# fbcotter/pytorch_wavelets

Hardware: AMD Instinct MI355X
Metric: Mpixels/s fwd+inv DWT J=3 db4, Nx3x512x512 fp32; % HBM roofline (higher is better)
Workload: dtype f32; 1 GPU; DWTForward+DWTInverse J=3 db4 symmetric, 128x3x512x512 fp32 per GPU (BASELINE configs[1]); global_batch=128, parallelism=batch-sharded x1, no data-path collective, step=forward + inverse

## Files before the change

include/wavelets_hip.h:

```cpp
#ifndef WAVELETS_HIP_H
#define WAVELETS_HIP_H
#include <stdint.h>

#ifdef __cplusplus
extern "C" {
#endif

#define WL_F32 0
#define WL_F16 1
#define WL_F64 2
#define WL_BF16 3

#define WL_ERR_MODE (-1)
#define WL_ERR_SHAPE (-2)
#define WL_ERR_UNSUPPORTED (-3)
#define WL_ERR_DTYPE (-4)
#define WL_ERR_TAPS (-5)
#define WL_MAX_TAPS 128

int wl_version(void);
const char* wl_backend(void);

int wl_set_option(const char* name, int value);
int wl_get_option(const char* name);
const char* wl_last_kernel(void);
long long wl_launch_count(void);
long long wl_last_grid(void);
const char* wl_kernel_history(int back);

int wl_dwt_coeff_len(int n, int L, int mode);

int wl_dwt2d_analysis(const void* x, void* ll, void* highs, int dtype, int64_t planes, int H, int W,
                      const void* h_w_lo, const void* h_w_hi, int Lw,
                      const void* h_h_lo, const void* h_h_hi, int Lh, int mode, void* stream);

int wl_dwt2d_analysis_strided(const void* x, int64_t x_plane_stride, int x_row_stride, void* ll,
                              int64_t ll_plane_stride, int ll_row_stride, void* highs, int dtype, int64_t planes,
                              int H, int W, const void* h_w_lo, const void* h_w_hi, int Lw, const void* h_h_lo,
                              const void* h_h_hi, int Lh, int mode, void* stream);

int wl_dwt2d_synthesis(const void* ll, int64_t ll_plane_stride, int ll_row_stride, const void* highs,
                       void* y, int dtype, int64_t planes, int Kh, int Kw, int OH, int OW,
                       const void* g_w_lo, const void* g_w_hi, int Lw,
                       const void* g_h_lo, const void* g_h_hi, int Lh, int mode, void* stream);

int wl_dwt2d_analysis_fused(const void* x, void* yl, void* const* yh, int dtype, int64_t planes, int H,
                            int W, int nlev, const void* h_w_lo, const void* h_w_hi, const void* h_h_lo,
                            const void* h_h_hi, int L, int mode, int strips, void* stream);
int wl_dwt2d_analysis_fused_ex(const void* x, int64_t x_plane_stride, int x_row_stride, void* yl, void* const* yh,
                               int dtype, int64_t planes, int H, int W, int nlev, const void* h_w_lo,
                               const void* h_w_hi, const void* h_h_lo, const void* h_h_hi, int L, int mode,
                               int strips, void* tap_scratch, int* tap_state, void* stream);

int wl_dwt2d_synthesis_fused(const void* yl, int64_t yl_plane_stride, int yl_row_stride, int yl_h, int yl_w,
                             const void* const* yh, const int* Kh, const int* Kw, void* y, int dtype,
                             int64_t planes, int nlev, const void* g_w_lo, const void* g_w_hi,
                             const void* g_h_lo, const void* g_h_hi, int L, int mode, int strips, void* stream);
int wl_dwt2d_synthesis_fused_ex(const void* yl, int64_t yl_plane_stride, int yl_row_stride, int yl_h, int yl_w,
                                const void* const* yh, const int* Kh, const int* Kw, void* y, int dtype,
                                int64_t planes, int nlev, const void* g_w_lo, const void* g_w_hi,
                                const void* g_h_lo, const void* g_h_hi, int L, int mode, int strips, void* tap_scratch,
                                int* tap_state, void* stream);

int wl_dwt2d_analysis_nonsep(const void* x, void* y, int dtype, int64_t planes, int H, int W, const void* f,
                             int Ly, int Lx, int mode, void* stream);
int wl_dwt2d_synthesis_nonsep(const void* coeffs, void* y, int dtype, int64_t planes, int Kh, int Kw, int OH,
                              int OW, const void* g, int Ly, int Lx, int mode, void* stream);


int wl_dtcwt_fwd_level1(const void* x, void* ll, void* highs, int dtype, int64_t planes, int H, int W,
                        const void* h0, int L0, const void* h1, int L1, int mode, void* stream);

int wl_dtcwt_fwd_level2(const void* x, void* ll, void* highs, int dtype, int64_t planes, int H, int W,
                        const void* h0a, const void* h0b, const void* h1a, const void* h1b, int L, void* stream);

int wl_dtcwt_fwd_level12(const void* x, void* highs1, void* ll2, void* highs2, int dtype, int64_t planes, int H, int W,
                         const void* h0o, int L0, const void* h1o, int L1, const void* h0a, const void* h0b,
                         const void* h1a, const void* h1b, int LQ, int mode, int policy, void* stream);

int wl_dtcwt_inv_level21(const void* ll2, int64_t ll2_plane_stride, int ll2_row_stride, const void* highs2,
                         const void* highs1, void* y, int dtype, int64_t planes, int H, int W, const void* g0o, int L0,
                         const void* g1o, int L1, const void* g0a, const void* g0b, const void* g1a, const void* g1b, int LQ,
                         int mode, int policy, void* stream);

int wl_dtcwt_inv_level1(const void* ll, int64_t ll_plane_stride, int ll_row_stride, const void* highs, void* y,
                        int dtype, int64_t planes, int H, int W, const void* g0, int L0, const void* g1, int L1,
                        int mode, void* stream);

int wl_dtcwt_inv_level2(const void* ll, int64_t ll_plane_stride, int ll_row_stride, const void* highs, void* y,
                        int dtype, int64_t planes, int h, int w, const void* g0a, const void* g0b, const void* g1a,
                        const void* g1b, int L, void* stream);

int wl_scat_fwd_level1(const void* x, void* z, void* drdx, void* drdy, void* ll, int dtype, int64_t N, int C, int H,
                       int W, const void* h0, int L0, const void* h1, int L1, int mode, double magbias,
                       int combine_colour, void* stream);

int wl_scat_fwd_level1_into(const void* x, void* z, int64_t z_batch_stride, int64_t z_ll_offset, int64_t z_mag_offset,
                            void* ll, int dtype, int64_t N, int C, int H, int W, const void* h0, int L0, const void* h1,
                            int L1, int mode, double magbias, void* stream);
int wl_scat_fwd_level2_into(const void* x, void* z, int64_t z_batch_stride, int64_t z_ll_offset, int64_t z_mag_offset,
                            int dtype, int64_t N, int C, int H, int W, const void* h0a, const void* h0b, const void* h1a,
                            const void* h1b, int L, double magbias, void* stream);

int wl_scat_bwd_level1(const void* dz, const void* drdx, const void* drdy, void* dx, int dtype, int64_t N, int C,
                       int H, int W, const void* h0, int L0, const void* h1, int L1, int mode, int combine_colour,
                       void* stream);

#define WL_TAP_SCRATCH_BYTES 64
int wl_dwt2d_analysis_stream(const void* x, int64_t x_plane_stride, int x_row_stride, void* ll, int64_t ll_plane_stride,
                             int ll_row_stride, void* highs, int dtype, int64_t planes, int H, int W, const void* h_w_lo,
                             const void* h_w_hi, const void* h_h_lo, const void* h_h_hi, int L, int mode, int policy,
                             void* stream);
int wl_dwt2d_analysis_stream_ex(const void* x, int64_t x_plane_stride, int x_row_stride, void* ll, int64_t ll_plane_stride,
                                int ll_row_stride, void* highs, int dtype, int64_t planes, int H, int W, const void* h_w_lo,
                                const void* h_w_hi, const void* h_h_lo, const void* h_h_hi, int L, int mode, int policy,
                                void* tap_scratch, int* tap_state, void* stream);

int wl_dwt2d_synthesis_stream(const void* ll, int64_t ll_plane_stride, int ll_row_stride, const void* highs, void* y,
                              int dtype, int64_t planes, int Kh, int Kw, int OH, int OW, const void* g_w_lo,
                              const void* g_w_hi, const void* g_h_lo, const void* g_h_hi, int L, int mode, int policy,
                              void* stream);
int wl_dwt2d_synthesis_stream_ex(const void* ll, int64_t ll_plane_stride, int ll_row_stride, const void* highs, void* y,
                                 int dtype, int64_t planes, int Kh, int Kw, int OH, int OW, const void* g_w_lo,
                                 const void* g_w_hi, const void* g_h_lo, const void* g_h_hi, int L, int mode, int policy,
                                 void* tap_scratch, int* tap_state, void* stream);

int wl_dwt2d_analysis_nonsep_bwd(const void* dy, void* dx, int dtype, int64_t planes, int H, int W, const void* f,
                                 int Ly, int Lx, int mode, void* stream);
int wl_dwt2d_synthesis_nonsep_bwd(const void* dy, void* dc, int dtype, int64_t planes, int Kh, int Kw, const void* g,
                                  int Ly, int Lx, int mode, void* stream);

int wl_dwt1d_analysis_fused(const void* x, void* lo, void* const* highs, int dtype, int64_t rows, int N, int J,
                            const void* h0, const void* h1, int L, int mode, void* stream);

int wl_dwt1d_synthesis_fused(const void* lo, int n_lo, const void* const* highs, const int* n_hi, void* y, int out_len, int dtype,
                             int64_t rows, int J, const void* g0, const void* g1, int L, int mode, void* stream);

int wl_corr1d(const void* x, void* y0, void* y1, int dtype, int64_t outer, int n, int64_t inner, int64_t y_outer_stride,
              int K, const void* h0, const void* h1, int tap_offset, int tap_stride, int ntaps, int start, int step,
              int tap_step, int ext, int out_offset, int out_stride, void* stream);

int wl_dwt2d_analysis_small(const void* x, void* yl, void* const* yh, int dtype, int64_t planes, int H, int W, int nlev,
                            const void* h_w_lo, const void* h_w_hi, const void* h_h_lo, const void* h_h_hi, int L, int mode,
                            void* stream);

int wl_dwt2d_synthesis_small(const void* yl, int yl_h, int yl_w, const void* const* yh, const int* Kh, const int* Kw, void* y,
                             int dtype, int64_t planes, int nlev, const void* g_w_lo, const void* g_w_hi, const void* g_h_lo,
                             const void* g_h_hi, int L, int mode, void* stream);

int wl_dtcwt_fwd_level1_rot(const void* x, void* ll, void* re, void* im, int dtype, int64_t N, int C, int H, int W,
                            const void* h0, int L0, const void* h1, int L1, const void* h2, int L2, int mode,
                            int scat, double magbias, void* stream);

int wl_swt2d_level(const void* x, int64_t x_ps, void* y, int dtype, int64_t planes, int H, int W,
                   const void* h_w_lo, const void* h_w_hi, const void* h_h_lo, const void* h_h_hi, int Lw, int Lh,
                   int dilation, int ext, void* stream);

int wl_iswt2d_level(const void* y, int64_t y_ps, const void* ll, int64_t ll_ps, int ll_mode, void* x, int dtype, int64_t planes,
                    int H, int W, const void* h_w_lo, const void* h_w_hi, const void* h_h_lo, const void* h_h_hi, int Lw, int Lh,
                    int dilation, int ext, double scale, void* stream);

int wl_corr1d_adj(const void* y0, int64_t y0_outer_stride, const void* y1, int64_t y1_outer_stride, void* dx, int dtype,
                  int64_t outer, int n, int64_t inner, int K, const void* h0, const void* h1, int ntaps, int start, int tap_step,
                  int ext, double scale, void* stream);

int wl_synth1d(const void* lo, const void* hi, void* y, int dtype, int64_t outer, int K, int64_t inner, int ny,
               const void* g0, const void* g1, int L, int mode, void* stream);

#ifdef __cplusplus
}
#endif
#endif
```

pytorch_wavelets_amd/_capi.py:

```python
import ctypes as C

P = C.c_void_p
I = C.c_int
L = C.c_int64

PROTOTYPES = {
    'wl_version': (I, []),
    'wl_backend': (C.c_char_p, []),
    'wl_set_option': (I, [C.c_char_p, I]),
    'wl_get_option': (I, [C.c_char_p]),
    'wl_last_kernel': (C.c_char_p, []),
    'wl_launch_count': (C.c_longlong, []),
    'wl_last_grid': (C.c_longlong, []),
    'wl_kernel_history': (C.c_char_p, [I]),
    'wl_dwt_coeff_len': (I, [I, I, I]),
    'wl_dwt2d_analysis': (I, [P, P, P, I, L, I, I, P, P, I, P, P, I, I, P]),
    'wl_dwt2d_analysis_strided': (I, [P, L, I, P, L, I, P, I, L, I, I, P, P, I, P, P, I, I, P]),
    'wl_dwt2d_synthesis': (I, [P, L, I, P, P, I, L, I, I, I, I, P, P, I, P, P, I, I, P]),
    'wl_dwt2d_analysis_fused': (I, [P, P, C.POINTER(P), I, L, I, I, I, P, P, P, P, I, I, I, P]),
    'wl_dwt2d_analysis_fused_ex': (I, [P, L, I, P, C.POINTER(P), I, L, I, I, I, P, P, P, P, I, I, I, P, C.POINTER(I), P]),
    'wl_dwt2d_synthesis_fused': (I, [P, L, I, I, I, C.POINTER(P), C.POINTER(I), C.POINTER(I), P, I, L, I, P, P, P, P, I, I, I, P]),
    'wl_dwt2d_synthesis_fused_ex': (I, [P, L, I, I, I, C.POINTER(P), C.POINTER(I), C.POINTER(I), P, I, L, I, P, P, P, P, I, I, I, P, C.POINTER(I), P]),
    'wl_dwt2d_analysis_stream': (I, [P, L, I, P, L, I, P, I, L, I, I, P, P, P, P, I, I, I, P]),
    'wl_dwt2d_analysis_stream_ex': (I, [P, L, I, P, L, I, P, I, L, I, I, P, P, P, P, I, I, I, P, C.POINTER(I), P]),
    'wl_dwt2d_synthesis_stream': (I, [P, L, I, P, P, I, L, I, I, I, I, P, P, P, P, I, I, I, P]),
    'wl_dwt2d_synthesis_stream_ex': (I, [P, L, I, P, P, I, L, I, I, I, I, P, P, P, P, I, I, I, P, C.POINTER(I), P]),
    'wl_dwt2d_analysis_nonsep': (I, [P, P, I, L, I, I, P, I, I, I, P]),
    'wl_dwt2d_synthesis_nonsep': (I, [P, P, I, L, I, I, I, I, P, I, I, I, P]),
    'wl_dwt2d_analysis_nonsep_bwd': (I, [P, P, I, L, I, I, P, I, I, I, P]),
    'wl_dwt2d_synthesis_nonsep_bwd': (I, [P, P, I, L, I, I, P, I, I, I, P]),
    'wl_dtcwt_fwd_level1': (I, [P, P, P, I, L, I, I, P, I, P, I, I, P]),
    'wl_dtcwt_fwd_level2': (I, [P, P, P, I, L, I, I, P, P, P, P, I, P]),
    'wl_dtcwt_fwd_level12': (I, [P, P, P, P, I, L, I, I, P, I, P, I, P, P, P, P, I, I, I, P]),
    'wl_dtcwt_inv_level21': (I, [P, L, I, P, P, P, I, L, I, I, P, I, P, I, P, P, P, P, I, I, I, P]),
    'wl_dtcwt_inv_level1': (I, [P, L, I, P, P, I, L, I, I, P, I, P, I, I, P]),
    'wl_dtcwt_inv_level2': (I, [P, L, I, P, P, I, L, I, I, P, P, P, P, I, P]),
    'wl_scat_fwd_level1': (I, [P, P, P, P, P, I, L, I, I, I, P, I, P, I, I, C.c_double, I, P]),
    'wl_scat_fwd_level1_into': (I, [P, P, L, L, L, P, I, L, I, I, I, P, I, P, I, I, C.c_double, P]),
    'wl_scat_fwd_level2_into': (I, [P, P, L, L, L, I, L, I, I, I, P, P, P, P, I, C.c_double, P]),
    'wl_dwt1d_analysis_fused': (I, [P, P, C.POINTER(P), I, L, I, I, P, P, I, I, P]),
    'wl_dwt2d_analysis_small': (I, [P, P, C.POINTER(P), I, L, I, I, I, P, P, P, P, I, I, P]),
    'wl_dwt2d_synthesis_small': (I, [P, I, I, C.POINTER(P), C.POINTER(I), C.POINTER(I), P, I, L, I, P, P, P, P, I, I, P]),
    'wl_dtcwt_fwd_level1_rot': (I, [P, P, P, P, I, L, I, I, I, P, I, P, I, P, I, I, I, C.c_double, P]),
    'wl_swt2d_level': (I, [P, L, P, I, L, I, I, P, P, P, P, I, I, I, I, P]),
    'wl_iswt2d_level': (I, [P, L, P, L, I, P, I, L, I, I, P, P, P, P, I, I, I, I, C.c_double, P]),
    'wl_dwt1d_synthesis_fused': (I, [P, I, C.POINTER(P), C.POINTER(I), P, I, I, L, I, P, P, I, I, P]),
    'wl_corr1d': (I, [P, P, P, I, L, I, L, L, I, P, P, I, I, I, I, I, I, I, I, I, P]),
    'wl_corr1d_adj': (I, [P, L, P, L, P, I, L, I, L, I, P, P, I, I, I, I, C.c_double, P]),
    'wl_synth1d': (I, [P, P, P, I, L, I, L, I, P, P, I, I, P]),
    'wl_scat_bwd_level1': (I, [P, P, P, P, I, L, I, I, I, P, I, P, I, I, I, P]),
}


def bind(lib):
    for name, (res, args) in PROTOTYPES.items():
        fn = getattr(lib, name)
        fn.restype = res
        fn.argtypes = args
    return lib
```

pytorch_wavelets_amd/csrc/wl_api_common.h:

```cpp
#pragma once
#include <stdlib.h>
#include "../../include/wavelets_hip.h"
#include "wl_common.h"
#include "wl_lattice.h"

static int wl_mode_to_ext(int mode) {
    switch (mode) {
        case 0: return WL_EXT_ZERO;
        case 1: return WL_EXT_SYM;
        case 2: return WL_EXT_PER;
        case 4: return WL_EXT_REFL;
        case 6: return WL_EXT_PERIODIC;
        default: return -1;
    }
}

static inline int wl_coeff_len(int n, int L, int mode) { return mode == 2 ? (n + 1) / 2 : (n + L - 1) / 2; }

static int wl_afb_base(int n, int L, int mode) {
    if (mode == 2) return L / 2 - L + 1;
    const int K = (n + L - 1) / 2;
    const int p = 2 * (K - 1) - n + L;
    return -(p / 2);
}

struct WlBanks { const void* w_lo; const void* w_hi; const void* h_lo; const void* h_hi; };
struct WlAfbReq {
    const void* x; int64_t x_ps; int x_rs;
    void* ll; int64_t ll_ps; int ll_rs; void* highs;
    int64_t planes; int H, W;
    WlBanks taps; int Lw, Lh, mode;
    int policy; float* scratch; int* tstate; void* stream;
};
struct WlSfbReq {
    const void* ll; int64_t ll_ps; int ll_rs; const void* highs; void* y;
    int64_t planes; int Kh, Kw, OH, OW;
    WlBanks taps; int Lw, Lh, mode;
    int policy; float* scratch; int* tstate; void* stream;
};
struct WlAfbPyrReq {
    const void* x; int64_t x_ps; int x_rs;
    void* yl; void* const* yh;
    int64_t planes; int H, W, nlev;
    WlBanks taps; int L, mode;
    int strips, hints; float* scratch; int* tstate; void* stream;
};
struct WlSfbPyrReq {
    const void* yl; int64_t yl_ps; int yl_rs; int yl_h, yl_w;
    const void* const* yh; const int* Kh; const int* Kw; void* y;
    int64_t planes; int nlev;
    WlBanks taps; int L, mode;
    int strips, hints; float* scratch; int* tstate; void* stream;
};

#define WL_DISPATCH_DTYPE(dtype, ...)                      \
    switch (dtype) {                                       \
        case WL_F32: { typedef float T; __VA_ARGS__; } break;    \
        case WL_F16: { typedef wl_half T; __VA_ARGS__; } break;  \
        case WL_BF16: { typedef wl_bf16 T; __VA_ARGS__; } break; \
        case WL_F64: { typedef double T; __VA_ARGS__; } break;   \
        default: return WL_ERR_DTYPE;                      \
    }
#define WL_DISPATCH_FLOAT(dtype, ...)                                      \
    do {                                                                   \
        if ((dtype) == WL_F32) { typedef float T; __VA_ARGS__; }           \
        if ((dtype) == WL_F16) { typedef wl_half T; __VA_ARGS__; }         \
        if ((dtype) == WL_BF16) { typedef wl_bf16 T; __VA_ARGS__; }        \
        return (dtype) == WL_F64 ? WL_ERR_UNSUPPORTED : WL_ERR_DTYPE;      \
    } while (0)

#define WL_GUARDED_PAIR(HINT, PLAIN, ...)                         \
    do {                                                          \
        int rc_ = PLAIN(__VA_ARGS__, 2, 1);                       \
        if (rc_ != 0) return rc_;                                 \
        rc_ = HINT(__VA_ARGS__, 1, 0);                            \
        if (rc_ != 0) return rc_;                                 \
        return PLAIN(__VA_ARGS__, 2, 2);                          \
    } while (0)

template <int LT, typename Plain, typename Lattice>
static int wl_lattice_launch(Plain plain, Lattice lattice, const WlBanks& b, int syn, int same, size_t elem_size,
                             float* scratch, int* tstate, int bits, void* stream) {
    int rc = plain(2, 1);
    if (rc != 0) return rc;
    rc = lattice(1, 1);
    if (rc != 0) return rc;
    WlTapPrepArgs p;
    p.h_w_lo = (const float*)b.w_lo; p.h_w_hi = (const float*)b.w_hi; p.h_h_lo = (const float*)b.h_lo; p.h_h_hi = (const float*)b.h_hi;
    p.out = scratch; p.L = LT; p.syn = syn; p.same = same;
    p.tol = elem_size == 2 ? 0x1p-12f : 0x1p-22f;
    rc = wl_tap_examined(tstate, bits) ? 0 : wl_launch_aux<WlTapPrep<LT> >(p, 1, 0, stream);
    if (rc != 0) return rc;
    wl_tap_mark(tstate, bits);
    rc = lattice(1, 0);
    if (rc != 0) return rc;
    return plain(2, 2);
}
```

pytorch_wavelets_amd/csrc/wl_idwt_rows.h:

```cpp
#pragma once
#include "wl_common.h"
#include "wl_dwt_rows.h"
#include "wl_lattice.h"

#define WL_IROWS_MAXLEV 3
#define WL_IROWS_WAVES 14
#define WL_IROWS_MAXHB 640
#ifndef WL_IROWS_ABLATE
#define WL_IROWS_ABLATE 0
#endif
#if (WL_IROWS_ABLATE & 8) && defined(__HIPCC__)
#define WL_ITICK() __builtin_readcyclecounter()
#else
#define WL_ITICK() 0ull
#endif
#define WL_IROWS_CHUNK 1024

struct WlIRowsLevel {
    int Kh, Kw;
    int OH, OW;
    int src_off[4];
    int ll_rows;
    int ll_pitch;
    int rbytes;
    int dma_rows;
    int dma_shift;
    int cpr;
    int nwaves;
    int per_d0, head_off;
    int per_grp;
};

struct WlIRowsSeg {
    int nhb;
    int f0[WL_IROWS_MAXLEV], fend[WL_IROWS_MAXLEV];
    int rho[WL_IROWS_MAXLEV];
    int own_lo, own_hi;
    unsigned sched[WL_IROWS_MAXHB / 4];
};

template <typename T>
struct WlIRowsArgs {
    const T* yl;
    const T* yh[WL_IROWS_MAXLEV];
    T* y;
    const float* g_w_lo;
    const float* g_w_hi;
    const float* g_h_lo;
    const float* g_h_hi;
    int64_t NC, ll_ps;
    int nlev, nwhole, lds_bytes;
    signed char role_level[WL_IROWS_WAVES];
    short role_arg[WL_IROWS_WAVES];
    signed char role_sub[WL_IROWS_WAVES];
    int pp, lds_plane;
    WlIRowsLevel g[WL_IROWS_MAXLEV];
    WlIRowsSeg seg[3];
    int per;
    int guard;
    const float* lat;
};

struct WlIRowsSched {
    int fed[WL_IROWS_MAXLEV];
    WL_HD void init(const WlIRowsSeg& sg) { for (int j = 0; j < WL_IROWS_MAXLEV; ++j) fed[j] = sg.f0[j]; }
    WL_HD int made(const WlIRowsSeg& sg, int j, int LT) const {
        const int warm = (LT - 2) / 2;
        return fed[j] - sg.f0[j] > warm ? 2 * (fed[j] - warm) : 2 * sg.f0[j];
    }
    template <typename A> WL_HD int feeds_now(const A& a, const WlIRowsSeg& sg, int j, int LT) const {
        const int warm = (LT - 2) / 2;
        int n = 0;
        while (n < 2 && fed[j] + n < sg.fend[j]) {
            const int k = fed[j] + n;
            if (j + 1 < a.nlev && k >= made(sg, j + 1, LT) && !(a.per && k >= a.g[j].Kh)) break;
            if (j > 0 && k - sg.f0[j] >= warm && 2 * (k - warm) + 1 - a.g[j - 1].ll_rows >= fed[j - 1]) break;
            ++n;
        }
        return n;
    }
};

#ifndef WL_IROWS_LAT_MIN
#define WL_IROWS_LAT_MIN 8
#endif
template <typename T, int LT, int LAT = 0, int PER = 0>
struct WlSfbRows {
    typedef WlIRowsArgs<T> Args;
    static const int kThreads = 64 * WL_IROWS_WAVES;
    static const int kMinWaves = 7;
    static const int HL = LT / 2;
    static const int WARM = HL - 1;
    static const int SZ = (int)sizeof(T);

    static WL_DEV void loader(const Args& a, const WlIRowsSeg& sg, const WlCtx& ctx, int64_t plane, int lane, int j, int s0, int ns, int soff) {
        const WlIRowsLevel& g = a.g[j];
        const int rb = g.rbytes, R = g.dma_rows, cpr = g.cpr;
        const int plane_bytes = g.Kh * rb, ring_bytes = R * rb;
        const int f0 = sg.f0[j], fend = sg.fend[j];
        const int r0 = f0 >> g.dma_shift;
        const char* src[4];
        int dst[4];
#pragma unroll
        for (int i = 0; i < 4; ++i) {
            const int s = s0 + (i < ns ? i : 0);
            src[i] = s == 0 ? reinterpret_cast<const char*>(a.yl + (size_t)plane * a.ll_ps)
                            : reinterpret_cast<const char*>(a.yh[j] + ((size_t)plane * 3 + (s - 1)) * ((size_t)g.Kh * g.Kw));
            dst[i] = g.src_off[s] + soff;
        }
        auto need = [&](int k) { return ((k >> g.dma_shift) - r0) * cpr + (((k & (R - 1)) + 1) * rb - 1) / WL_IROWS_CHUNK + 1; };
        const int total = fend > f0 ? need(fend - 1) : 0;
        const int max_steps = WL_IROWS_MAX_VM / ns - 1;
        const int p16 = plane_bytes & ~15, ptail = (plane_bytes & 15) / 4;
        int issued = 0, landed = 0;
        int r = r0, c = 0;
        int rbyte = 0, pbyte = r0 * ring_bytes;
        int fed = f0;
        auto try_issue = [&]() {
            if (issued >= total || issued - landed >= max_steps) return false;
            const int cend = rbyte + WL_IROWS_CHUNK < ring_bytes ? rbyte + WL_IROWS_CHUNK : ring_bytes;
            if (r != r0 && cend > (fed - 2 - (r - 1) * R) * rb) return false;
            if (!(WL_IROWS_ABLATE & 2)) {
                const bool whole = pbyte + 16 <= plane_bytes;
                const bool on = rbyte + lane * 16 < ring_bytes && pbyte + lane * 16 + 16 <= plane_bytes;
                const bool tail = ptail && p16 >= pbyte && p16 < pbyte + (cend - rbyte);
#pragma unroll
                for (int i = 0; i < 4; ++i) {
                    if (i >= ns) break;
                    if (whole) wl_dma16_s(ctx, (unsigned)(dst[i] + rbyte), src[i], (unsigned)(pbyte + lane * 16), on);
                    if (tail) wl_dma4_s(ctx, (unsigned)(dst[i] + rbyte + (p16 - pbyte)), src[i], (unsigned)(p16 + lane * 4), lane < ptail);
                }
            }
            ++issued;
            rbyte += WL_IROWS_CHUNK; pbyte += WL_IROWS_CHUNK;
            if (++c == cpr) { c = 0; ++r; rbyte = 0; pbyte = r * ring_bytes; }
            return true;
        };
        while (try_issue()) {}
        unsigned long long tw = 0, tb = 0, ti = 0;
        unsigned word = sg.sched[0];
        for (int hb = 0; hb < sg.nhb; ++hb) {
            const unsigned long long c0 = WL_ITICK();
            const int n = (int)(word >> (8 * (hb & 3) + 2 * j)) & 3;
            if ((hb & 3) == 3) word = sg.sched[(hb >> 2) + 1 < WL_IROWS_MAXHB / 4 ? (hb >> 2) + 1 : 0];
            if (n) {
                const int nd = need(fed + n - 1);
                if (issued < nd) wl_fail();
                if (!(WL_IROWS_ABLATE & 2)) wl_wait_vm_dyn((issued - nd) * ns);
                landed = nd;
            }
            const unsigned long long c1 = WL_ITICK();
            if (!(WL_IROWS_ABLATE & 64) || !(hb & 1)) ctx.sync();
            const unsigned long long c2 = WL_ITICK();
            fed += n;
            while (try_issue()) {}
            tw += c1 - c0; tb += c2 - c1; ti += WL_ITICK() - c2;
        }
        wl_wait_vm<0>();
        if ((WL_IROWS_ABLATE & 8) && lane == 0) {
            T* o = a.y + (size_t)plane * a.g[0].OH * a.g[0].OW + 4 * (ctx.tid >> 6);
            o[0] = (T)(float)(tw >> 6); o[1] = (T)(float)(tb >> 6); o[2] = (T)(float)(ti >> 6);
        }
    }

    static WL_DEV void loader_per(const Args& a, const WlIRowsSeg& sg, const WlCtx& ctx, int64_t plane, int lane, int j, int s0, int ns, int soff) {
        const WlIRowsLevel& g = a.g[j];
        const int P = g.rbytes, R = g.dma_rows, Kh = g.Kh, rowb = g.Kw * SZ;
        const int rowb16 = rowb & ~15, tail = (rowb & 15) / 4;
        const int nseg = (rowb16 + WL_IROWS_CHUNK - 1) / WL_IROWS_CHUNK;
        const int per_row = ns * (nseg + (tail ? 1 : 0));
        const int f0 = sg.f0[j], fend = sg.fend[j], rho = sg.rho[j];
        const char* src[4];
        int dst[4];
#pragma unroll
        for (int i = 0; i < 4; ++i) {
            const int s = s0 + (i < ns ? i : 0);
            src[i] = s == 0 ? reinterpret_cast<const char*>(a.yl + (size_t)plane * a.ll_ps)
                            : reinterpret_cast<const char*>(a.yh[j] + ((size_t)plane * 3 + (s - 1)) * ((size_t)g.Kh * g.Kw));
            dst[i] = g.src_off[s] + soff;
        }
        const int G = g.per_grp;
        const int per_step = G > 1 ? ns : per_row;
        const int lrg = (16 * lane) / P, lo = 16 * lane - lrg * P - g.per_d0;
        const bool lon = lrg < G && lo >= 0 && lo + 16 <= rowb;
        const int fend_g = (fend + G - 1) & ~(G - 1);
        const int max_rows = (WL_IROWS_MAX_VM / per_step - 1) * G;
        int next = f0, landed = f0;
        int fed = f0;
        auto try_issue = [&]() {
            if (next >= fend_g || next - landed >= max_rows) return false;
            if (next + G - 1 - R >= fed - 2) return false;
            if (G > 1) {
                int sr = next + lrg - WARM + rho;
                sr = sr < 0 ? sr + Kh : sr;
                sr = sr >= Kh ? sr - Kh : sr;
                sr = sr >= Kh ? sr - Kh : sr;
                const unsigned gro = (unsigned)sr * (unsigned)rowb + (unsigned)lo;
                const unsigned slot = (unsigned)((next & (R - 1)) * P);
                if (!(WL_IROWS_ABLATE & 2)) {
#pragma unroll
                    for (int i = 0; i < 4; ++i) {
                        if (i >= ns) break;
                        wl_dma16_s(ctx, (unsigned)dst[i] + slot, src[i], gro, lon);
                    }
                }
                next += G;
                return true;
            }
            int sr = next - WARM + rho;
            sr = sr < 0 ? sr + Kh : sr;
            sr = sr >= Kh ? sr - Kh : sr;
            const unsigned gro = (unsigned)sr * (unsigned)rowb;
            const unsigned slot = (unsigned)((next & (R - 1)) * P + g.per_d0);
            if (!(WL_IROWS_ABLATE & 2)) {
#pragma unroll
                for (int i = 0; i < 4; ++i) {
                    if (i >= ns) break;
                    for (int q = 0; q < nseg; ++q) {
                        const int byte = (q * 64 + lane) * 16;
                        wl_dma16_s(ctx, (unsigned)dst[i] + slot + (unsigned)(q * WL_IROWS_CHUNK), src[i], gro + (unsigned)byte, byte + 16 <= rowb);
                    }
                    if (tail) wl_dma4_s(ctx, (unsigned)dst[i] + slot + (unsigned)rowb16, src[i], gro + (unsigned)(rowb16 + lane * 4), lane < tail);
                }
            }
            ++next;
            return true;
        };
        while (try_issue()) {}
        unsigned word = sg.sched[0];
        for (int hb = 0; hb < sg.nhb; ++hb) {
            const int n = (int)(word >> (8 * (hb & 3) + 2 * j)) & 3;
            if ((hb & 3) == 3) word = sg.sched[(hb >> 2) + 1 < WL_IROWS_MAXHB / 4 ? (hb >> 2) + 1 : 0];
            if (n) {
                const int nd = (fed + n + G - 1) & ~(G - 1);
                if (next < nd) wl_fail();
                if (!(WL_IROWS_ABLATE & 2)) wl_wait_vm_dyn(G > 1 ? ((next - nd) / G) * per_step : (next - nd) * per_step);
                landed = nd;
                if (WARM > 0) {
                    for (int it = lane; it < n * ns * WARM; it += 64) {
                        const int h = it % WARM, rs = it / WARM, i = rs % ns, rr = rs / ns;
                        char* row = ctx.smem + (dst[i < 4 ? i : 0] + ((fed + rr) & (R - 1)) * P + g.per_d0);
                        *reinterpret_cast<T*>(row + (h - WARM) * SZ) = *reinterpret_cast<const T*>(row + (g.Kw - WARM + h) * SZ);
                    }
                }
            }
            ctx.sync();
            fed += n;
            while (try_issue()) {}
        }
        wl_wait_vm<0>();
    }

    struct __attribute__((packed, aligned(sizeof(T)), may_alias)) WlPairT { T a, b; };
    static const int NP = (HL + 1) / 2;
    static const int NW = HL > 1 ? HL - 1 : 1;
    struct Wave {
        wl_v2 gw0[HL], gw1[LAT ? 1 : HL], gh0[LAT ? 1 : HL], gh1[LAT ? 1 : HL];
        wl_v2 lt[LAT ? HL : 1];
        int coff;
        int coff_ll;
        int ycol1;
        int hcol0, hcol1;
        int rot2, xoh;
        int lhead;
        int llmask;
        bool two;
        bool odd_wave;
        char* yp; unsigned yrowb, ycol;
        int lring, lpitch, lmask, lrows, lcol;
    };

    static WL_DEV void load_coeffs(const char* p, wl_v2 (&v)[NP]) {
#pragma unroll
        for (int i = 0; i < HL / 2; ++i)
            v[i] = wl_v2{(float)*reinterpret_cast<const T*>(p + 2 * i * SZ), (float)*reinterpret_cast<const T*>(p + (2 * i + 1) * SZ)};
        if (HL & 1) v[NP - 1] = wl_v2{(float)*reinterpret_cast<const T*>(p + (HL - 1) * SZ), 0.f};
    }
    static WL_DEV void row_syn(const WlIRowsLevel& g, const Wave& R, const char* smem, int k, wl_v2& na, wl_v2& nb) {
        int rll = g.src_off[0] + (k & R.llmask) * g.ll_pitch;
        if (PER && g.head_off >= 0 && k >= g.Kh) rll = g.head_off + (k - g.Kh) * g.ll_pitch;
        const int rb = (k & (g.dma_rows - 1)) * g.rbytes;
        wl_v2 vll[NP], vlh[NP], vhl[NP], vhh[NP];
        load_coeffs(smem + (rll + (PER ? R.coff_ll : R.coff)), vll);
        load_coeffs(smem + (g.src_off[1] + rb + R.coff), vlh);
        load_coeffs(smem + (g.src_off[2] + rb + R.coff), vhl);
        load_coeffs(smem + (g.src_off[3] + rb + R.coff), vhh);
        na = wl_pk_mul_x(R.gw0[HL - 1], vll[0]);
        nb = wl_pk_mul_x(R.gw0[HL - 1], vlh[0]);
        if constexpr (LAT != 0) {
            wl_qmf_syn_fma<0>(na, R.gw0[0], vhl[0]);
            wl_qmf_syn_fma<0>(nb, R.gw0[0], vhh[0]);
#pragma unroll
            for (int u = 1; u < HL; ++u) {
                const int t = HL - 1 - u;
                if (u & 1) {
                    wl_pk_fma_y(na, R.gw0[t], vll[u / 2]); wl_pk_fma_y(nb, R.gw0[t], vlh[u / 2]);
                    wl_qmf_syn_fma<1>(na, R.gw0[u], vhl[u / 2]); wl_qmf_syn_fma<1>(nb, R.gw0[u], vhh[u / 2]);
                } else {
                    wl_pk_fma_x(na, R.gw0[t], vll[u / 2]); wl_pk_fma_x(nb, R.gw0[t], vlh[u / 2]);
                    wl_qmf_syn_fma<0>(na, R.gw0[u], vhl[u / 2]); wl_qmf_syn_fma<0>(nb, R.gw0[u], vhh[u / 2]);
                }
            }
            return;
        }
        wl_pk_fma_x(na, R.gw1[LAT ? 0 : HL - 1], vhl[0]);
        wl_pk_fma_x(nb, R.gw1[LAT ? 0 : HL - 1], vhh[0]);
#pragma unroll
        for (int u = 1; u < HL; ++u) {
            const int t = LAT ? 0 : HL - 1 - u;
            if (u & 1) {
                wl_pk_fma_y(na, R.gw0[t], vll[u / 2]); wl_pk_fma_y(nb, R.gw0[t], vlh[u / 2]);
                wl_pk_fma_y(na, R.gw1[t], vhl[u / 2]); wl_pk_fma_y(nb, R.gw1[t], vhh[u / 2]);
            } else {
                wl_pk_fma_x(na, R.gw0[t], vll[u / 2]); wl_pk_fma_x(nb, R.gw0[t], vlh[u / 2]);
                wl_pk_fma_x(na, R.gw1[t], vhl[u / 2]); wl_pk_fma_x(nb, R.gw1[t], vhh[u / 2]);
            }
        }
    }
    static WL_DEV void lat_feed(const Wave& R, wl_v2 (&S)[NW], wl_v2 a, wl_v2 b, wl_v2& y0, wl_v2& y1) {
        wl_v2 q = wl_fma_s<0, 1>(a, R.lt[HL - 1], b);
        wl_v2 p = wl_fma_s<0, 0>(b, R.lt[HL - 1], a);
#pragma unroll
        for (int k = HL - 1; k >= 1; --k) {
            const wl_v2 d = S[k - 1];
            S[k - 1] = q;
            const wl_v2 n = wl_fma_s<1, 0>(d, R.lt[k - 1], p);
            q = wl_fma_s<0, 0>(p, R.lt[k - 1], d);
            p = n;
        }
        y0 = wl_v2{p.x, q.x}; y1 = wl_v2{p.y, q.y};
    }
    template <int OFF, int NE>
    static WL_DEV void col_syn(const Wave& R, const wl_v2 (&ea)[NE], const wl_v2 (&eb)[NE], wl_v2& y0, wl_v2& y1) {
        y0 = wl_pk_mul_x(R.gh0[0], ea[OFF + HL - 1]); y1 = wl_pk_mul_y(R.gh0[0], ea[OFF + HL - 1]);
        wl_pk_fma_x(y0, R.gh1[0], eb[OFF + HL - 1]);
        wl_pk_fma_y(y1, R.gh1[0], eb[OFF + HL - 1]);
#pragma unroll
        for (int t = 1; t < HL; ++t) {
            wl_pk_fma_x(y0, R.gh0[LAT ? 0 : t], ea[OFF + HL - 1 - t]);
            wl_pk_fma_y(y1, R.gh0[LAT ? 0 : t], ea[OFF + HL - 1 - t]);
            wl_pk_fma_x(y0, R.gh1[LAT ? 0 : t], eb[OFF + HL - 1 - t]);
            wl_pk_fma_y(y1, R.gh1[LAT ? 0 : t], eb[OFF + HL - 1 - t]);
        }
    }
    template <int j>
    static WL_DEV void emit_per(const Wave& R, char* smem, int m, wl_v2 y0, wl_v2 y1) {
        if (j == 0) {
            if ((WL_IROWS_ABLATE & 1) && y0.x + y0.y + y1.x + y1.y != 1.2345e30f) return;
            int r0 = m + R.rot2;
            r0 = r0 < 0 ? r0 + R.xoh : r0;
            r0 = r0 >= R.xoh ? r0 - R.xoh : r0;
            int r1 = r0 + 1;
            r1 = r1 >= R.xoh ? r1 - R.xoh : r1;
            char* p0 = R.yp + (unsigned)r0 * R.yrowb;
            char* p1 = R.yp + (unsigned)r1 * R.yrowb;
            if (!R.odd_wave) {
                T v[2] = {(T)y0.x, (T)y1.x}, w[2] = {(T)y0.y, (T)y1.y};
                *reinterpret_cast<WlPairT*>(p0 + R.ycol) = *reinterpret_cast<WlPairT*>(v);
                *reinterpret_cast<WlPairT*>(p1 + R.ycol) = *reinterpret_cast<WlPairT*>(w);
            } else {
                *reinterpret_cast<T*>(p0 + R.ycol) = (T)y0.x; *reinterpret_cast<T*>(p0 + R.ycol1) = (T)y1.x;
                *reinterpret_cast<T*>(p1 + R.ycol) = (T)y0.y; *reinterpret_cast<T*>(p1 + R.ycol1) = (T)y1.y;
            }
        } else {
#pragma unroll
            for (int rr = 0; rr < 2; ++rr) {
                const int row = m + rr;
                if (row >= R.lrows) continue;
                const T va = (T)(rr ? y0.y : y0.x), vb = (T)(rr ? y1.y : y1.x);
                char* d = smem + (R.lring + (row & R.lmask) * R.lpitch);
                T v[2] = {va, vb};
                *reinterpret_cast<WlPairT*>(d + R.lcol) = *reinterpret_cast<WlPairT*>(v);
                if (R.hcol0 >= 0) *reinterpret_cast<T*>(d + R.hcol0) = va;
                if (R.hcol1 >= 0) *reinterpret_cast<T*>(d + R.hcol1) = vb;
                if (row < WARM) {
                    char* h = smem + (R.lhead + row * R.lpitch);
                    *reinterpret_cast<WlPairT*>(h + R.lcol) = *reinterpret_cast<WlPairT*>(v);
                    if (R.hcol0 >= 0) *reinterpret_cast<T*>(h + R.hcol0) = va;
                    if (R.hcol1 >= 0) *reinterpret_cast<T*>(h + R.hcol1) = vb;
                }
            }
        }
    }
    template <int j>
    static WL_DEV void emit(const Wave& R, char* smem, int m, wl_v2 y0, wl_v2 y1) {
        if constexpr (PER != 0) { emit_per<j>(R, smem, m, y0, y1); return; }
        if (j == 0) {
            if ((WL_IROWS_ABLATE & 1) && y0.x + y0.y + y1.x + y1.y != 1.2345e30f) return;
            char* r0 = R.yp + ((unsigned)m * R.yrowb + R.ycol);
            char* r1 = r0 + R.yrowb;
            if (!R.odd_wave) {
#if (WL_STREAM_NT & 2) && defined(__HIPCC__)
                typedef T WlVec2 __attribute__((ext_vector_type(2), aligned(sizeof(T))));
                WlVec2 v = {(T)y0.x, (T)y1.x}, w = {(T)y0.y, (T)y1.y};
                __builtin_nontemporal_store(v, reinterpret_cast<WlVec2*>(r0));
                __builtin_nontemporal_store(w, reinterpret_cast<WlVec2*>(r1));
#else
                T v[2] = {(T)y0.x, (T)y1.x}, w[2] = {(T)y0.y, (T)y1.y};
                *reinterpret_cast<WlPairT*>(r0) = *reinterpret_cast<WlPairT*>(v);
                *reinterpret_cast<WlPairT*>(r1) = *reinterpret_cast<WlPairT*>(w);
#endif
            } else {
                *reinterpret_cast<T*>(r0) = (T)y0.x;
                *reinterpret_cast<T*>(r1) = (T)y0.y;
                if (R.two) { *reinterpret_cast<T*>(r0 + SZ) = (T)y1.x; *reinterpret_cast<T*>(r1 + SZ) = (T)y1.y; }
            }
        } else {
            if (m < R.lrows) {
                T v[2] = {(T)y0.x, (T)y1.x};
                *reinterpret_cast<WlPairT*>(smem + (R.lring + (m & R.lmask) * R.lpitch + R.lcol)) = *reinterpret_cast<WlPairT*>(v);
            }
            if (m + 1 < R.lrows) {
                T v[2] = {(T)y0.y, (T)y1.y};
                *reinterpret_cast<WlPairT*>(smem + (R.lring + ((m + 1) & R.lmask) * R.lpitch + R.lcol)) = *reinterpret_cast<WlPairT*>(v);
            }
        }
    }

    template <int j>
    static WL_DEV void compute(const Args& a, const WlIRowsSeg& sg, const WlCtx& ctx, int64_t plane, int c0, int lane, int soff) {
        const WlIRowsLevel& g = a.g[j];
        char* const smem = ctx.smem + soff;
        const int c = c0 + lane;
        const bool active = 2 * c < g.OW;
        Wave R;
        if constexpr (LAT != 0) {
            const float gsc = a.lat[1];
#pragma unroll
            for (int t = 0; t < HL; ++t) {
                R.gw0[t] = wl_uniform_v2(wl_v2{a.g_w_lo[2 * t] * gsc, a.g_w_lo[2 * t + 1] * gsc});
                R.lt[t] = wl_uniform_v2(wl_v2{a.lat[2 + t], -a.lat[2 + t]});
            }
        } else {
#pragma unroll
            for (int t = 0; t < HL; ++t) {
                R.gw0[t] = wl_uniform_v2(wl_v2{a.g_w_lo[2 * t], a.g_w_lo[2 * t + 1]});
                R.gw1[t] = wl_uniform_v2(wl_v2{a.g_w_hi[2 * t], a.g_w_hi[2 * t + 1]});
                R.gh0[t] = wl_uniform_v2(wl_v2{a.g_h_lo[2 * t], a.g_h_lo[2 * t + 1]});
                R.gh1[t] = wl_uniform_v2(wl_v2{a.g_h_hi[2 * t], a.g_h_hi[2 * t + 1]});
            }
        }
        R.coff = (active ? c : 0) * SZ;
        R.llmask = g.ll_rows - 1;
        R.two = 2 * c + 1 < g.OW;
        R.odd_wave = wl_uniform((g.OW & 1) && 2 * (c0 + 63) + 1 >= g.OW) != 0;
        R.yp = reinterpret_cast<char*>(a.y + (size_t)plane * g.OH * g.OW);
        R.yrowb = (unsigned)g.OW * SZ; R.ycol = (unsigned)(2 * c) * SZ;
        R.lmask = j > 0 ? a.g[j > 0 ? j - 1 : 0].ll_rows - 1 : 0;
        R.lring = j > 0 ? a.g[j > 0 ? j - 1 : 0].src_off[0] : 0;
        R.lpitch = j > 0 ? a.g[j > 0 ? j - 1 : 0].ll_pitch : 0;
        R.lrows = j > 0 ? a.g[j > 0 ? j - 1 : 0].Kh : 0;
        R.lcol = 2 * c * SZ;
        R.coff_ll = R.coff; R.ycol1 = 0; R.hcol0 = R.hcol1 = -1; R.rot2 = 0; R.xoh = g.OH; R.lhead = 0;
        if constexpr (PER != 0) {
            const int q = active ? c : 0;
            R.coff = g.per_d0 - WARM * SZ + q * SZ;
            R.coff_ll = j + 1 < a.nlev ? q * SZ : R.coff;
            if (j == 0) {
                int x0 = 2 * q - WARM;
                x0 = x0 < 0 ? x0 + g.OW : x0;
                int x1 = x0 + 1;
                x1 = x1 >= g.OW ? x1 - g.OW : x1;
                R.ycol = (unsigned)x0 * SZ; R.ycol1 = x1 * SZ;
                const int qs = (WARM - 1) / 2;
                R.odd_wave = (WARM & 1) && c0 <= qs && qs < c0 + 64;
                R.rot2 = 2 * sg.rho[0] - WARM;
            } else {
                const WlIRowsLevel& gl = a.g[j > 0 ? j - 1 : 0];
                R.lhead = gl.head_off;
                R.hcol0 = active && 2 * q < WARM ? (gl.Kw + 2 * q) * SZ : -1;
                R.hcol1 = active && 2 * q + 1 < WARM ? (gl.Kw + 2 * q + 1) * SZ : -1;
            }
        }
        wl_v2 wa[NW], wb[NW];
#pragma unroll
        for (int t = 0; t < NW; ++t) wa[t] = wb[t] = wl_v2{0.f, 0.f};
        const int f0 = sg.f0[j];
        int fed = f0;
        unsigned long long tb = 0, tf = 0, c2 = WL_ITICK();
        unsigned word = sg.sched[0];
        for (int hb = 0; hb < sg.nhb; ++hb) {
            const int n = (int)(word >> (8 * (hb & 3) + 2 * j)) & 3;
            if ((hb & 3) == 3) word = sg.sched[(hb >> 2) + 1 < WL_IROWS_MAXHB / 4 ? (hb >> 2) + 1 : 0];
            const unsigned long long c0 = WL_ITICK();
            if (!(WL_IROWS_ABLATE & 64) || !(hb & 1)) ctx.sync();
            const unsigned long long c1 = WL_ITICK();
            tf += c0 - c2; tb += c1 - c0; c2 = c1;
            if (n == 0) continue;
            const int k = fed;
            fed += n;
            if (!active || (WL_IROWS_ABLATE & 4)) continue;
            const int m = 2 * (k - WARM);
            wl_v2 y0, y1;
            if constexpr (LAT != 0) {
                wl_v2 na, nb;
                row_syn(g, R, smem, k, na, nb);
                lat_feed(R, wa, na, nb, y0, y1);
                if (k - f0 >= WARM) emit<j>(R, smem, m, y0, y1);
                if (n == 2) {
                    row_syn(g, R, smem, k + 1, na, nb);
                    lat_feed(R, wa, na, nb, y0, y1);
                    if (k + 1 - f0 >= WARM) emit<j>(R, smem, m + 2, y0, y1);
                }
                continue;
            }
            if (n == 2) {
                wl_v2 ea[HL + 1], eb[HL + 1];
                row_syn(g, R, smem, k, ea[HL - 1], eb[HL - 1]);
                row_syn(g, R, smem, k + 1, ea[HL], eb[HL]);
#pragma unroll
                for (int t = 0; t < HL - 1; ++t) { ea[t] = wa[t]; eb[t] = wb[t]; }
                if (k - f0 >= WARM) { col_syn<0>(R, ea, eb, y0, y1); emit<j>(R, smem, m, y0, y1); }
                if (k + 1 - f0 >= WARM) { col_syn<1>(R, ea, eb, y0, y1); emit<j>(R, smem, m + 2, y0, y1); }
#pragma unroll
                for (int t = 0; t < HL - 1; ++t) { wa[t] = ea[t + 2]; wb[t] = eb[t + 2]; }
            } else {
                wl_v2 ea[HL], eb[HL];
                row_syn(g, R, smem, k, ea[HL - 1], eb[HL - 1]);
#pragma unroll
                for (int t = 0; t < HL - 1; ++t) { ea[t] = wa[t]; eb[t] = wb[t]; }
                if (k - f0 >= WARM) { col_syn<0>(R, ea, eb, y0, y1); emit<j>(R, smem, m, y0, y1); }
#pragma unroll
                for (int t = 0; t < HL - 1; ++t) { wa[t] = ea[t + 1]; wb[t] = eb[t + 1]; }
            }
        }
        if ((WL_IROWS_ABLATE & 8) && lane == 0) {
            T* o = a.y + (size_t)plane * a.g[0].OH * a.g[0].OW + 4 * (ctx.tid >> 6);
            o[0] = (T)(float)(tb >> 6); o[1] = (T)(float)(tf >> 6); o[2] = (T)0;
        }
    }

    static WL_DEV void run(const Args& a, const WlCtx& ctx) {
        const int tid = ctx.tid;
        const int wave = wl_uniform(tid >> 6), lane = tid & 63;
        if (LT >= WL_IROWS_LAT_MIN && a.guard) {
            const bool holds = a.lat && *reinterpret_cast<const unsigned*>(a.lat) == WL_LAT_OK;
            if (!wl_guard_pass(a.guard, holds)) return;
        }
        const int64_t bid = ctx.bid;
        const int sub = wl_uniform(a.role_sub[wave]);
        const int64_t plane = (bid < a.nwhole ? bid : a.nwhole + (bid - a.nwhole) / 2) * a.pp + sub;
        const WlIRowsSeg& sg = a.seg[bid < a.nwhole ? 0 : 1 + (int)((bid - a.nwhole) & 1)];
        const int soff = sub * a.lds_plane;
        const int lev = plane < a.NC ? wl_uniform(a.role_level[wave]) : -2, arg = wl_uniform(a.role_arg[wave]);
        if (lev == -1) {
#if defined(__HIPCC__)
            __builtin_amdgcn_s_setprio(3);
#endif
            if constexpr (PER != 0) loader_per(a, sg, ctx, plane, lane, arg >> 4, (arg >> 2) & 3, (arg & 3) + 1, soff);
            else loader(a, sg, ctx, plane, lane, arg >> 4, (arg >> 2) & 3, (arg & 3) + 1, soff);
        }
        else if (lev == 0) compute<0>(a, sg, ctx, plane, arg, lane, soff);
        else if (lev == 1) compute<1>(a, sg, ctx, plane, arg, lane, soff);
        else if (lev == 2) compute<2>(a, sg, ctx, plane, arg, lane, soff);
        else
            for (int hb = 0; hb < sg.nhb; ++hb) if (!(WL_IROWS_ABLATE & 64) || !(hb & 1)) ctx.sync();
    }
};
```

pytorch_wavelets_amd/csrc/wl_lattice.h:

```cpp
#pragma once
#include "wl_common.h"

#define WL_LAT_MAXK 10
#define WL_TAP_SCRATCH_FLOATS 16
#define WL_LAT_OK 0x4c415431u

template <int L>
WL_HD bool wl_lattice_factor(const float* lo, const float* hi, double tol, float* g, float* T, bool syn = false) {
    static_assert(L >= 4 && L % 2 == 0 && L / 2 <= WL_LAT_MAXK, "even tap counts from 4 to 20");
    const int K = L / 2;
    double E[K][2][2], n0[K][2], n1[K][2], Td[K];
    double scale = 0.0;
#pragma unroll
    for (int i = 0; i < K; ++i) {
        const int e = syn ? 2 * i : L - 2 - 2 * i;
        E[i][0][0] = lo[e]; E[i][0][1] = lo[e + 1];
        E[i][1][0] = hi[e]; E[i][1][1] = hi[e + 1];
    }
#pragma unroll
    for (int t = 0; t < L; ++t) {
        const double a = lo[t] < 0 ? -(double)lo[t] : (double)lo[t], b = hi[t] < 0 ? -(double)hi[t] : (double)hi[t];
        if (!(a <= 1e30) || !(b <= 1e30)) return false;
        scale = a > scale ? a : scale; scale = b > scale ? b : scale;
    }
    if (!(scale > 0.0)) return false;
    auto ab = [](double v) { return v < 0 ? -v : v; };
    double res = 0.0, gain = 1.0;
#pragma unroll
    for (int k = K - 1; k >= 1; --k) {
        const int j = ab(E[k][0][0]) + ab(E[k][1][0]) >= ab(E[k][0][1]) + ab(E[k][1][1]) ? 0 : 1;
        const double x = E[k][0][j], y = E[k][1][j];
        const double r = __builtin_sqrt(x * x + y * y);
        if (!(r > 1e-12 * scale)) return false;
        const double s = x / r, c = y / r;
        if (!(ab(c) > 1e-7)) return false;
#pragma unroll
        for (int i = 0; i < K; ++i)
#pragma unroll
            for (int q = 0; q < 2; ++q) {
                if (i > k) continue;
                n0[i][q] = c * E[i][0][q] - s * E[i][1][q];
                n1[i][q] = s * E[i][0][q] + c * E[i][1][q];
            }
#pragma unroll
        for (int q = 0; q < 2; ++q) {
            res = ab(n0[k][q]) > res ? ab(n0[k][q]) : res;
            res = ab(n1[0][q]) > res ? ab(n1[0][q]) : res;
        }
#pragma unroll
        for (int i = 0; i < K - 1; ++i)
#pragma unroll
            for (int q = 0; q < 2; ++q) {
                if (i >= k) continue;
                E[i][0][q] = n0[i][q]; E[i][1][q] = n1[i + 1][q];
            }
        Td[k] = -(s / c);
        gain *= c;
    }
    const double c0 = E[0][1][1], s0 = E[0][1][0];
    res = ab(E[0][0][0] + c0) > res ? ab(E[0][0][0] + c0) : res;
    res = ab(E[0][0][1] - s0) > res ? ab(E[0][0][1] - s0) : res;
    if (!(ab(c0) > 1e-7)) return false;
    Td[0] = -(s0 / c0);
    gain *= c0;
    if (!(res <= tol * scale)) return false;
#pragma unroll
    for (int k = 0; k < K; ++k) {
        if (!(ab(Td[k]) < 1e6)) return false;
        T[k] = (float)Td[k];
    }
    *g = (float)(-gain);
    return ab(gain) > 1e-30;
}

template <int HI, int NZ> WL_DEV wl_v2 wl_fma_s(wl_v2 w, wl_v2 pair, wl_v2 z) {
    wl_v2 d;
#if defined(__HIPCC__)
    if (!HI && !NZ) asm("v_pk_fma_f32 %0, %1, %2, %3 op_sel_hi:[1,0,1]" : "=v"(d) : "v"(w), "s"(pair), "v"(z));
    else if (HI && !NZ) asm("v_pk_fma_f32 %0, %1, %2, %3 op_sel:[0,1,0] op_sel_hi:[1,1,1]" : "=v"(d) : "v"(w), "s"(pair), "v"(z));
    else if (!HI && NZ) asm("v_pk_fma_f32 %0, %1, %2, %3 op_sel_hi:[1,0,1] neg_lo:[0,0,1] neg_hi:[0,0,1]" : "=v"(d) : "v"(w), "s"(pair), "v"(z));
    else asm("v_pk_fma_f32 %0, %1, %2, %3 op_sel:[0,1,0] op_sel_hi:[1,1,1] neg_lo:[0,0,1] neg_hi:[0,0,1]" : "=v"(d) : "v"(w), "s"(pair), "v"(z));
#else
    const float c = HI ? pair.y : pair.x;
    d.x = __builtin_fmaf(w.x, c, NZ ? -z.x : z.x); d.y = __builtin_fmaf(w.y, c, NZ ? -z.y : z.y);
#endif
    return d;
}

template <int LT> WL_DEV void wl_qmf_fma(wl_v2& acc, const wl_v2 (&bank)[LT / 2], int t, int xy, wl_v2 s) {
    const int u = t < LT / 2 ? t : LT - 1 - t;
    const bool sw = t >= LT / 2, neg = t & 1;
#if defined(__HIPCC__)
    if (!sw && !neg) { if (xy) asm("v_pk_fma_f32 %0, %1, %2, %0 op_sel:[0,1,0] op_sel_hi:[1,1,1]" : "+v"(acc) : "s"(bank[u]), "v"(s));
                       else asm("v_pk_fma_f32 %0, %1, %2, %0 op_sel_hi:[1,0,1]" : "+v"(acc) : "s"(bank[u]), "v"(s)); }
    else if (!sw && neg) { if (xy) asm("v_pk_fma_f32 %0, %1, %2, %0 op_sel:[0,1,0] op_sel_hi:[1,1,1] neg_hi:[1,0,0]" : "+v"(acc) : "s"(bank[u]), "v"(s));
                           else asm("v_pk_fma_f32 %0, %1, %2, %0 op_sel_hi:[1,0,1] neg_hi:[1,0,0]" : "+v"(acc) : "s"(bank[u]), "v"(s)); }
    else if (sw && !neg) { if (xy) asm("v_pk_fma_f32 %0, %1, %2, %0 op_sel:[1,1,0] op_sel_hi:[0,1,1]" : "+v"(acc) : "s"(bank[u]), "v"(s));
                           else asm("v_pk_fma_f32 %0, %1, %2, %0 op_sel:[1,0,0] op_sel_hi:[0,0,1]" : "+v"(acc) : "s"(bank[u]), "v"(s)); }
    else { if (xy) asm("v_pk_fma_f32 %0, %1, %2, %0 op_sel:[1,1,0] op_sel_hi:[0,1,1] neg_hi:[1,0,0]" : "+v"(acc) : "s"(bank[u]), "v"(s));
           else asm("v_pk_fma_f32 %0, %1, %2, %0 op_sel:[1,0,0] op_sel_hi:[0,0,1] neg_hi:[1,0,0]" : "+v"(acc) : "s"(bank[u]), "v"(s)); }
#else
    const float c = xy ? s.y : s.x;
    const float lo = sw ? bank[u].y : bank[u].x, hi = (sw ? bank[u].x : bank[u].y) * (neg ? -1.f : 1.f);
    acc.x = __builtin_fmaf(lo, c, acc.x); acc.y = __builtin_fmaf(hi, c, acc.y);
#endif
}
template <int LT> WL_DEV wl_v2 wl_qmf_mul(const wl_v2 (&bank)[LT / 2], int t, int xy, wl_v2 s) {
    const int u = t < LT / 2 ? t : LT - 1 - t;
    const bool sw = t >= LT / 2, neg = t & 1;
    wl_v2 r;
#if defined(__HIPCC__)
    if (!sw && !neg) { if (xy) asm("v_pk_mul_f32 %0, %1, %2 op_sel:[0,1] op_sel_hi:[1,1]" : "=v"(r) : "s"(bank[u]), "v"(s));
                       else asm("v_pk_mul_f32 %0, %1, %2 op_sel_hi:[1,0]" : "=v"(r) : "s"(bank[u]), "v"(s)); }
    else if (!sw && neg) { if (xy) asm("v_pk_mul_f32 %0, %1, %2 op_sel:[0,1] op_sel_hi:[1,1] neg_hi:[1,0]" : "=v"(r) : "s"(bank[u]), "v"(s));
                           else asm("v_pk_mul_f32 %0, %1, %2 op_sel_hi:[1,0] neg_hi:[1,0]" : "=v"(r) : "s"(bank[u]), "v"(s)); }
    else if (sw && !neg) { if (xy) asm("v_pk_mul_f32 %0, %1, %2 op_sel:[1,1] op_sel_hi:[0,1]" : "=v"(r) : "s"(bank[u]), "v"(s));
                           else asm("v_pk_mul_f32 %0, %1, %2 op_sel:[1,0] op_sel_hi:[0,0]" : "=v"(r) : "s"(bank[u]), "v"(s)); }
    else { if (xy) asm("v_pk_mul_f32 %0, %1, %2 op_sel:[1,1] op_sel_hi:[0,1] neg_hi:[1,0]" : "=v"(r) : "s"(bank[u]), "v"(s));
           else asm("v_pk_mul_f32 %0, %1, %2 op_sel:[1,0] op_sel_hi:[0,0] neg_hi:[1,0]" : "=v"(r) : "s"(bank[u]), "v"(s)); }
#else
    const float c = xy ? s.y : s.x;
    const float lo = sw ? bank[u].y : bank[u].x, hi = (sw ? bank[u].x : bank[u].y) * (neg ? -1.f : 1.f);
    r.x = lo * c; r.y = hi * c;
#endif
    return r;
}

template <int Y> WL_DEV void wl_qmf_syn_fma(wl_v2& acc, wl_v2 pair, wl_v2 sv) {
#if defined(__HIPCC__)
    if (Y) asm("v_pk_fma_f32 %0, %1, %2, %0 op_sel:[1,1,0] op_sel_hi:[0,1,1] neg_hi:[1,0,0]" : "+v"(acc) : "s"(pair), "v"(sv));
    else asm("v_pk_fma_f32 %0, %1, %2, %0 op_sel:[1,0,0] op_sel_hi:[0,0,1] neg_hi:[1,0,0]" : "+v"(acc) : "s"(pair), "v"(sv));
#else
    const float c = Y ? sv.y : sv.x;
    acc.x = __builtin_fmaf(pair.y, c, acc.x); acc.y = __builtin_fmaf(-pair.x, c, acc.y);
#endif
}

struct WlTapPrepArgs {
    const float* h_w_lo; const float* h_w_hi; const float* h_h_lo; const float* h_h_hi;
    float* out;
    int L;
    float tol;
    int syn;
    int same;
};
static inline bool wl_tap_examined(const int* st, int need) { return st && (*st & need) == need; }
static inline void wl_tap_mark(int* st, int bits) { if (st) *st |= bits; }

template <int LT>
struct WlTapPrep {
    typedef WlTapPrepArgs Args;
    static const int kThreads = 64;
    static const int kMinWaves = 1;
    static WL_DEV void run(const Args& a, const WlCtx& ctx) {
        if (ctx.bid != 0) return;
        float g = 0.f, T[LT / 2];
#pragma unroll
        for (int k = 0; k < LT / 2; ++k) T[k] = 0.f;
        bool ok = wl_taps_qmf(a.h_w_lo, a.h_w_hi, LT) && wl_taps_qmf(a.h_h_lo, a.h_h_hi, LT);
        if (a.same) ok = ok & wl_taps_same(a.h_w_lo, a.h_h_lo, LT) & wl_taps_same(a.h_w_hi, a.h_h_hi, LT);
        ok = wl_lattice_factor<LT>(a.h_h_lo, a.h_h_hi, (double)a.tol, &g, T, a.syn != 0) && ok;
        if (ctx.tid != 0) return;
        unsigned* flag = reinterpret_cast<unsigned*>(a.out);
        a.out[1] = g;
#pragma unroll
        for (int k = 0; k < LT / 2; ++k) a.out[2 + k] = T[k];
        flag[0] = ok ? WL_LAT_OK : 0u;
    }
};
```

pytorch_wavelets_amd/csrc/wl_rows_api.inc:

```
#include "wl_api_common.h"
#include "wl_dwt_rows.h"

#ifndef WL_ROWS_PACK_CUT
#define WL_ROWS_PACK_CUT 1
#endif
static int wl_rows_pack_and_cut(int64_t planes, int pp_cap, int lds_plane, int rows, int halo, int64_t cost_now, int64_t max_wgs) {
    if (!WL_ROWS_PACK_CUT) return 0;
    const int64_t cus = wl_num_cus(), slots = 2 * cus;
    int p2 = pp_cap < planes ? pp_cap : (int)planes;
    while (p2 > 1 && (p2 * lds_plane > 80 * 1024 || 8 * ((planes + p2 - 1) / p2) < 3 * cus)) --p2;
    if (p2 <= 1) return 0;
    const int64_t wgs = 2 * ((planes + p2 - 1) / p2);
    if (wgs > max_wgs) return 0;
    const int64_t cost = ((wgs + slots - 1) / slots) * (rows / 2 + halo + 8);
    return cost * 10 < cost_now * 9 ? p2 : 0;
}

#if !defined(WL_ROWS_UNIT_SYNTHESIS)
template <typename T>
static int wl_rows_plan_segment(const WlRowsArgs<T>& a, WlRowsSeg& sg, int LT, int* need) {
    const int nlev = a.nlev;
    WlRowsSched sc;
    sc.init(sg);
    for (int j = 0; j < WL_ROWS_MAXLEV; ++j) need[j] = 0;
    int nhb = 0;
    for (;; ++nhb) {
        int nn[WL_ROWS_MAXLEV], todo = 0;
        for (int j = 0; j < nlev; ++j) { nn[j] = sc.feeds_now(a, sg, j, LT); todo += sg.fend[j] - sc.fed[j]; }
        if (todo == 0) break;
        if (nhb >= WL_ROWS_MAXHB) return WL_ERR_UNSUPPORTED;
        if ((nhb & 3) == 0) sg.sched[nhb >> 2] = 0;
        int any = 0;
        for (int j = 0; j < nlev; ++j) { sg.sched[nhb >> 2] |= (unsigned)nn[j] << (8 * (nhb & 3) + 2 * j); any += nn[j]; }
        if (!any) return WL_ERR_UNSUPPORTED;
        for (int j = 0; j + 1 < nlev; ++j) {
            const int wr_hi = sc.avail(sg, j, LT) + nn[j];
            const int e_next = a.base + 2 * sc.fed[j + 1];
            const int e_last = a.base + 2 * sg.fend[j + 1] - 1;
            int oldest = a.g[j + 1].Hs;
            if (a.ext == WL_EXT_PER) oldest = e_next <= e_last ? e_next : 0x3fffffff;
            else if (e_next <= e_last) {
                const int cand[4] = {e_next, e_last, e_next < 0 ? -1 : e_next, e_next < 0 ? 0 : e_next};
                for (int c = 0; c < 4; ++c) {
                    if (cand[c] < e_next || cand[c] > e_last) continue;
                    const int r = wl_ext1(cand[c], a.g[j + 1].Hs, a.ext);
                    if (r >= 0 && r < oldest) oldest = r;
                }
            }
            if (wr_hi - oldest > need[j + 1]) need[j + 1] = wr_hi - oldest;
        }
        for (int j = 0; j < nlev; ++j) sc.fed[j] += nn[j];
    }
    sg.nhb = nhb;
    return 0;
}

#if defined(__HIPCC__)
#define WL_DECLINE(n) WL_ERR_UNSUPPORTED
#else
#include <stdio.h>
static int wl_decline_trace(int n, int line) {
    if (getenv("WL_EMU_TRACE")) fprintf(stderr, "[wl] fused analysis declined at check %d (wl_rows_api.inc:%d)\n", n, line);
    return WL_ERR_UNSUPPORTED;
}
#define WL_DECLINE(n) wl_decline_trace(n, __LINE__)
#endif
template <typename T, int LT, int PPR, int SAME = 0, int LAT = 0, int ODD = 0, int NP2 = 0>
static int wl_afb_rows_launch(const WlAfbPyrReq& r, const float* lat, int guard = 0, int what = 0) {
    typedef WlAfbRows<T, LT, PPR, WL_ROWS_DEPTH, SAME, LAT, ODD, NP2> K;
    const int WARM = (LT - 2) / 2;
    const int64_t planes = r.planes;
    const int H = r.H, W = r.W, nlev = r.nlev, mode = r.mode, strips = r.strips;
    WlRowsArgs<T> a;
    a.ext = wl_mode_to_ext(mode);
    const bool per = a.ext == WL_EXT_PER;
    if (nlev < 1 || nlev > WL_ROWS_MAXLEV) return WL_DECLINE(1);
    if (nlev > 1 && !(a.ext == WL_EXT_ZERO || a.ext == WL_EXT_SYM || a.ext == WL_EXT_REFL || per)) return WL_DECLINE(2);
    if ((int64_t)H * r.x_rs >= (1LL << 30) || r.x_rs < W) return WL_DECLINE(3);
    if ((r.x_rs * sizeof(T)) % 16 != 0 || (r.x_ps * sizeof(T)) % 16 != 0 || (uintptr_t)r.x % 16 != 0 || wl_cdiv(W * (int)sizeof(T), 1024) != PPR) return WL_DECLINE(4);
    if ((W * sizeof(T)) % 16 != 0 && wl_align_up(W * (int)sizeof(T), 16) > r.x_rs * (int)sizeof(T)) return WL_DECLINE(5);
    a.base = wl_afb_base(W, LT, mode);
    if ((a.base & 1) != ODD) return WL_DECLINE(6);
    a.nlev = nlev;
    int compute_waves = 0;
    {
        int h = H, w = W, wave = 0;
        for (int j = 0; j < nlev; ++j) {
            WlRowsLevel& g = a.g[j];
            g.Hs = h; g.Ws = w;
            if (per && (h + (h & 1) < LT - 1 || w + (w & 1) < LT - 1)) return WL_DECLINE(7);
            g.Kh = wl_coeff_len(h, LT, mode); g.Kw = wl_coeff_len(w, LT, mode);
            g.nwaves = wl_cdiv(g.Kw, 64); wave += g.nwaves;
            g.hl = (a.base < 0 ? -a.base : 0) + ODD;
            const int e_max = 2 * (g.Kw - 1) + a.base + LT - 1 + ODD;
            g.hr = e_max > w - 1 ? e_max - (w - 1) : 0;
            if (g.hl > w || g.hr > w || (4 / WL_ROWS_LOADERS) * (g.hl + g.hr) > 128) return WL_DECLINE(8);
            g.pad = wl_align_up(g.hl * (int)sizeof(T), 16);
            g.ring_pitch = wl_align_up(g.pad + (w + g.hr) * (int)sizeof(T), 16);
            if (j > 0) {
                const int e_last = a.base + 2 * (g.Kh + WARM) - 1;
                if (-a.base > h || e_last >= 2 * h - 1 || h < 2) return WL_DECLINE(9);
                if (per && ((h & 1) || (w & 1))) return WL_DECLINE(10);
            }
            h = g.Kh; w = g.Kw;
        }
        for (int j = nlev; j < WL_ROWS_MAXLEV; ++j) { a.g[j] = a.g[nlev - 1]; a.g[j].nwaves = 0; a.yh[j] = nullptr; }
        if (wave + WL_ROWS_LOADERS > WL_ROWS_WAVES) return WL_DECLINE(11);
        compute_waves = wave;
    }
    for (int t = 0; t < 3; ++t)
        for (int j = 0; j < WL_ROWS_MAXLEV; ++j) { a.seg[t].f0[j] = a.seg[t].fend[j] = a.seg[t].own_lo[j] = a.seg[t].own_hi[j] = 0; }
    bool can_split = true;
    {
        int F0[WL_ROWS_MAXLEV], FEND[WL_ROWS_MAXLEV];
        for (int j = nlev - 1; j >= 0; --j) {
            F0[j] = 0; FEND[j] = a.g[j].Kh + WARM;
            if (per && j + 1 < nlev) { F0[j] = a.base + 2 * F0[j + 1]; FEND[j] = a.base + 2 * FEND[j + 1] + WARM; }
        }
        int m[WL_ROWS_MAXLEV];
        m[nlev - 1] = a.g[nlev - 1].Kh / 2;
        for (int j = nlev - 2; j >= 0; --j) m[j] = a.base + 2 * m[j + 1];
        for (int j = 0; j < nlev; ++j) if (m[j] < 1 || m[j] >= a.g[j].Kh - 1) can_split = false;
        for (int j = 0; j < nlev; ++j) {
            const int Kh = a.g[j].Kh;
            a.seg[0].f0[j] = F0[j]; a.seg[0].fend[j] = FEND[j]; a.seg[0].own_lo[j] = 0; a.seg[0].own_hi[j] = Kh;
            if (!can_split) continue;
            a.seg[2].f0[j] = m[j]; a.seg[2].fend[j] = FEND[j]; a.seg[2].own_lo[j] = m[j]; a.seg[2].own_hi[j] = Kh;
            a.seg[1].f0[j] = F0[j]; a.seg[1].own_lo[j] = 0; a.seg[1].own_hi[j] = m[j];
        }
        if (can_split)
            for (int j = nlev - 1; j >= 0; --j) {
                int rows = a.seg[1].own_hi[j];
                if (j + 1 < nlev) {
                    const int need = a.base + 2 * a.seg[1].fend[j + 1];
                    if (need > rows) rows = need;
                }
                if (rows > FEND[j] - WARM) rows = FEND[j] - WARM;
                a.seg[1].fend[j] = rows + WARM;
            }
    }
    if (strips == 2 && !can_split) return WL_DECLINE(12);
    int off = 0;
    {
        int r0 = 8;
        while (r0 < LT) r0 *= 2;
        if (NP2) r0 = 2;
        for (int j = 0; j < WL_ROWS_MAXLEV; ++j) a.g[j].ring_rows = r0;
    }
    for (;;) {
        bool bad = false;
        for (int t = 0; t < (can_split ? 3 : 1) && !bad; ++t) {
            int need[WL_ROWS_MAXLEV];
            const int rc = wl_rows_plan_segment<T>(a, a.seg[t], LT, need);
            if (rc) { if (t == 0) return rc; can_split = false; break; }
            for (int j = 1; j < nlev; ++j)
                if (need[j] > a.g[j].ring_rows) {
                    if (NP2) a.g[j].ring_rows = need[j];
                    else a.g[j].ring_rows *= 2;
                    bad = true;
                    if (a.g[j].ring_rows > 64) return WL_DECLINE(13);
                }
        }
        if (!bad) break;
    }
    for (int j = 0; j < WL_ROWS_MAXLEV; ++j) a.g[j].ring_magic = (unsigned)(0x100000000ull / (unsigned)a.g[j].ring_rows);
    if (NP2)
        for (int j = 1; j < nlev; ++j) {
            const int rows = a.g[j].ring_rows, hi = a.g[j].Hs + 2 * LT + rows;
            int lo = a.base < 0 ? a.base : 0;
            if (-a.g[j].hl < lo) lo = -a.g[j].hl;
            if (-a.g[j - 1].hl < lo) lo = -a.g[j - 1].hl;
            unsigned long long seen = 0;
            for (int r = lo; r < lo + rows; ++r) seen |= 1ull << wl_ring_slot(r, rows, a.g[j].ring_magic);
            if (seen != (rows == 64 ? ~0ull : (1ull << rows) - 1)) return WL_DECLINE(16);
            for (int r = lo; r + rows <= hi; ++r)
                if (wl_ring_slot(r + rows, rows, a.g[j].ring_magic) != wl_ring_slot(r, rows, a.g[j].ring_magic)) return WL_DECLINE(16);
        }
    if (strips == 2 && !can_split) return WL_DECLINE(14);
    {
        int zero_bytes = 0;
        off = 0;
        for (int j = 0; j < nlev; ++j) {
            a.g[j].ring_off = off;
            off += (j == 0 ? 4 * K::NSLOT : a.g[j].ring_rows) * a.g[j].ring_pitch;
            if (a.g[j].ring_pitch > zero_bytes) zero_bytes = a.g[j].ring_pitch;
        }
        for (int j = nlev; j < WL_ROWS_MAXLEV; ++j) a.g[j].ring_off = a.g[nlev - 1].ring_off;
        a.zero_off = off; off += zero_bytes;
#if !defined(__HIPCC__)
        if (off > 80 * 1024 && getenv("WL_EMU_TRACE"))
            for (int j = 0; j < nlev; ++j) fprintf(stderr, "[wl]   level %d: ring rows %d pitch %d\n", j, j == 0 ? 4 * K::NSLOT : a.g[j].ring_rows, a.g[j].ring_pitch);
#endif
        if constexpr (!NP2 && !ODD && LT >= 12 && ((SAME && LAT) || (!SAME && !LAT))) {
            if (off > 80 * 1024 && nlev > 1)
                return wl_afb_rows_launch<T, LT, PPR, SAME, LAT, ODD, 1>(r, lat, guard, what);
        }
        if (off > 80 * 1024) return WL_DECLINE(15);
    }
    const int pp_cap = WL_ROWS_WAVES / (compute_waves + WL_ROWS_LOADERS);
    int pp = pp_cap;
    a.lds_plane = wl_align_up(off, 16);
    while (pp > 1 && (pp * a.lds_plane > 80 * 1024 || (planes + pp - 1) / pp < (int64_t)wl_num_cus())) --pp;
    if (strips == 2) pp = 1;
    bool pack_cut = false;
    if (strips == 0 && can_split && pp == 1 && pp_cap > 1) {
        const int64_t slots = 2 * (int64_t)wl_num_cus();
        const int p2 = wl_rows_pack_and_cut(planes, pp_cap, a.lds_plane, a.g[0].Kh, WARM, ((planes + slots - 1) / slots) * (int64_t)(a.g[0].Kh + 8), wl_num_cus());
        if (p2) { pp = p2; pack_cut = true; }
    }
    a.pp = pp;
    if (pp > 1) off = pp * a.lds_plane;
    a.lds_bytes = off;
    const int64_t units = (planes + pp - 1) / pp;
    int64_t ncut = 0;
    if (can_split && strips == 2) ncut = planes;
    else if (pack_cut) ncut = units;
    else if (can_split && strips == 0 && pp == 1) {
        const int64_t cus = wl_num_cus(), slots = 2 * cus;
        const int64_t rounds = (planes + slots - 1) / slots;
        ncut = rounds * slots - planes;
        if (ncut > planes) ncut = planes;
        if (rounds > 1 && ncut * 4 > planes) ncut = 0;
        if (planes <= cus) ncut = cus - planes < planes ? cus - planes : planes;
    }
    a.nwhole = (int)(units - ncut);
    {
        int load[4] = {0, 0, 0, 0}, cnt[4] = {0, 0, 0, 0};
        const int cap[4] = {(WL_ROWS_WAVES + 3) / 4, (WL_ROWS_WAVES + 2) / 4, (WL_ROWS_WAVES + 1) / 4, WL_ROWS_WAVES / 4};
        for (int w = 0; w < WL_ROWS_WAVES; ++w) { a.role_level[w] = -2; a.role_col0[w] = 0; a.role_sub[w] = 0; }
        int sub = 0;
        auto place = [&](int level, int col0, int cost) {
            int best = -1;
            for (int b = 0; b < 4; ++b)
                if (cnt[b] < cap[b] && (best < 0 || load[b] < load[best])) best = b;
            const int w = best + 4 * cnt[best];
            a.role_level[w] = (signed char)level; a.role_col0[w] = (short)col0; a.role_sub[w] = (signed char)sub;
            load[best] += cost; ++cnt[best];
        };
        for (sub = 0; sub < pp; ++sub)
            for (int j = 0; j < nlev; ++j)
                for (int c = 0; c < a.g[j].nwaves; ++c) place(j, 64 * c, 8 >> j);
        for (sub = 0; sub < pp; ++sub)
            for (int l = 0; l < WL_ROWS_LOADERS; ++l) place(-1, l, 4 / WL_ROWS_LOADERS);
    }
    a.x = (const T*)r.x; a.ll = (T*)r.yl;
    for (int j = 0; j < nlev; ++j) a.yh[j] = (T*)r.yh[j];
    a.h_w_lo = (const float*)r.taps.w_lo; a.h_w_hi = (const float*)r.taps.w_hi;
    a.h_h_lo = (const float*)r.taps.h_lo; a.h_h_hi = (const float*)r.taps.h_hi;
    a.NC = planes; a.x_ps = r.x_ps; a.x_rs = r.x_rs;
    a.ll_ps = (int64_t)a.g[nlev - 1].Kh * a.g[nlev - 1].Kw; a.ll_rs = a.g[nlev - 1].Kw;
    a.guard = guard;
    a.lat = lat;
    if (what == 1) return 0;
    return what == 2 ? wl_launch_armed<K>(a, units + ncut, (size_t)off, r.stream) : wl_launch<K>(a, units + ncut, (size_t)off, r.stream);
}

#ifndef WL_ROWS_LAT_MIN
#define WL_ROWS_LAT_MIN 10
#endif
template <typename T, int LT, int PPR, int ODD = 0>
static int wl_afb_rows_pick(const WlAfbPyrReq& r) {
    const bool same_hint = (r.hints & 1) != 0, qmf_hint = (r.hints & 2) != 0;
    const float* const none = nullptr;
    if constexpr (LT >= WL_ROWS_LAT_MIN) {
        if (same_hint && qmf_hint && r.scratch)
            return wl_lattice_launch<LT>([&](int guard, int what) { return wl_afb_rows_launch<T, LT, PPR, 0, 0, ODD>(r, r.scratch, guard, what); },
                                         [&](int guard, int what) { return wl_afb_rows_launch<T, LT, PPR, 1, 1, ODD>(r, r.scratch, guard, what); },
                                         r.taps, 0, 1, sizeof(T), r.scratch, r.tstate, 3, r.stream);
    }
    if constexpr (LT > 12) return WL_ERR_UNSUPPORTED;
    else {
        if constexpr (LT >= WL_ROWS_SAME_MIN && !ODD) {
            if (r.taps.w_lo == r.taps.h_lo && r.taps.w_hi == r.taps.h_hi) return wl_afb_rows_launch<T, LT, PPR, 1>(r, none);
            if (same_hint) WL_GUARDED_PAIR((wl_afb_rows_launch<T, LT, PPR, 1>), (wl_afb_rows_launch<T, LT, PPR, 0>), r, none);
        }
        return wl_afb_rows_launch<T, LT, PPR, 0, 0, ODD>(r, none);
    }
}

template <typename T>
static int wl_afb_rows_dispatch(const WlAfbPyrReq& r) {
    const int ppr = wl_cdiv(r.W * (int)sizeof(T), 1024);
    const bool odd = (wl_afb_base(r.W, r.L, r.mode) & 1) != 0;
#define WL_PICK(LT_, P_)                                                               \
    do {                                                                               \
        if constexpr (LT_ % 4 == 0) { if (odd) return wl_afb_rows_pick<T, LT_, P_, 1>(r); } \
        return wl_afb_rows_pick<T, LT_, P_, 0>(r);                                     \
    } while (0)
#define WL_CASE(LT_)                                                                   \
    case LT_:                                                                          \
        if (ppr == 1) WL_PICK(LT_, 1);                                                 \
        if (ppr == 2) WL_PICK(LT_, 2);                                                 \
        if constexpr (sizeof(T) == 4) {     \
            if (ppr == 3) WL_PICK(LT_, 3);                                             \
        }                                                                              \
        return WL_ERR_UNSUPPORTED
    switch (r.L) {
        WL_CASE(2); WL_CASE(4); WL_CASE(6); WL_CASE(8); WL_CASE(10); WL_CASE(12); WL_CASE(14); WL_CASE(16); WL_CASE(18); WL_CASE(20);
        default: return WL_ERR_UNSUPPORTED;
    }
#undef WL_CASE
#undef WL_PICK
}

extern "C" int wl_dwt2d_analysis_fused_ex(const void* xp, int64_t x_plane_stride, int x_row_stride, void* yl, void* const* yh,
                                          int dtype, int64_t planes, int H, int W, int nlev, const void* h_w_lo,
                                          const void* h_w_hi, const void* h_h_lo, const void* h_h_hi, int L, int mode,
                                          int strips, void* tap_scratch, int* tap_state, void* stream) {
    if (wl_mode_to_ext(mode) < 0) return WL_ERR_MODE;
    if (planes < 0 || H < 1 || W < 1 || x_row_stride < W || x_plane_stride < 0) return WL_ERR_SHAPE;
    if (L < 1 || L > WL_MAX_TAPS) return WL_ERR_TAPS;
    if (mode == 2 && (H + (H & 1) < L - 1 || W + (W & 1) < L - 1)) return WL_ERR_UNSUPPORTED;
    if (strips > 15) return WL_ERR_UNSUPPORTED;
    const int hints = strips < 0 ? 0 : ((strips & 4) ? 1 : 0) | ((strips & 8) ? 2 : 0);
    if (!tap_scratch) tap_state = nullptr;
    if (strips >= 0) strips &= 3;
    if (strips < 0 || strips > 2) return WL_ERR_UNSUPPORTED;
    if (strips == 0 && 8 * planes < 3 * wl_num_cus()) return WL_ERR_UNSUPPORTED;
    const WlAfbPyrReq r = {xp, x_plane_stride, x_row_stride, yl, yh, planes, H, W, nlev, {h_w_lo, h_w_hi, h_h_lo, h_h_hi}, L, mode,
                           strips, hints, (float*)tap_scratch, tap_state, stream};
    WL_DISPATCH_FLOAT(dtype, return planes == 0 ? 0 : wl_afb_rows_dispatch<T>(r));
}

extern "C" int wl_dwt2d_analysis_fused(const void* x, void* yl, void* const* yh, int dtype, int64_t planes,
                                       int H, int W, int nlev, const void* h_w_lo, const void* h_w_hi,
                                       const void* h_h_lo, const void* h_h_hi, int L, int mode, int strips, void* stream) {
    return wl_dwt2d_analysis_fused_ex(x, (int64_t)H * W, W, yl, yh, dtype, planes, H, W, nlev, h_w_lo, h_w_hi, h_h_lo, h_h_hi,
                                      L, mode, strips, nullptr, nullptr, stream);
}


#endif

#if !defined(WL_ROWS_UNIT_ANALYSIS)
#include "wl_idwt_rows.h"

template <typename T>
static int wl_irows_plan_segment(const WlIRowsArgs<T>& a, WlIRowsSeg& sg, int LT) {
    WlIRowsSched sc;
    sc.init(sg);
    int nhb = 0;
    for (;; ++nhb) {
        int nn[WL_IROWS_MAXLEV], todo = 0, any = 0;
        for (int j = 0; j < a.nlev; ++j) { nn[j] = sc.feeds_now(a, sg, j, LT); todo += sg.fend[j] - sc.fed[j]; any += nn[j]; }
        if (todo == 0) break;
        if (nhb >= WL_IROWS_MAXHB || !any) return WL_ERR_UNSUPPORTED;
        if ((nhb & 3) == 0) sg.sched[nhb >> 2] = 0;
        for (int j = 0; j < a.nlev; ++j) sg.sched[nhb >> 2] |= (unsigned)nn[j] << (8 * (nhb & 3) + 2 * j);
        for (int j = 0; j < a.nlev; ++j) sc.fed[j] += nn[j];
    }
    sg.nhb = nhb;
    return 0;
}

template <typename T, int LT, int LAT = 0, int PER = 0>
static int wl_sfb_rows_launch(const WlSfbPyrReq& r, const float* lat = nullptr, int guard = 0, int what = 0) {
    typedef WlSfbRows<T, LT, LAT, PER> K;
    const int SZ = (int)sizeof(T), WARM = K::WARM;
    const int64_t planes = r.planes, ll_ps = r.yl_ps;
    const int ll_rs = r.yl_rs, yl_h = r.yl_h, yl_w = r.yl_w, nlev = r.nlev, strips = r.strips;
    const void* const yl = r.yl; const void* const* const yh = r.yh;
    const int* const Kh = r.Kh; const int* const Kw = r.Kw;
    WlIRowsArgs<T> a;
    if (nlev < 1 || nlev > WL_IROWS_MAXLEV) return WL_ERR_UNSUPPORTED;
    a.nlev = nlev;
    a.per = PER;
    int compute_waves = 0;
    {
        int sh = yl_h, sw = yl_w;
        for (int j = nlev - 1; j >= 0; --j) {
            WlIRowsLevel& g = a.g[j];
            g.Kh = Kh[j]; g.Kw = Kw[j];
            if (g.Kh < LT / 2 || g.Kw < LT / 2) return WL_ERR_UNSUPPORTED;
            if (sh < g.Kh || sh > g.Kh + 1 || sw < g.Kw || sw > g.Kw + 1) return WL_ERR_SHAPE;
            if (PER && (sh != g.Kh || sw != g.Kw)) return WL_ERR_UNSUPPORTED;
            g.OH = PER ? 2 * g.Kh : 2 * g.Kh - LT + 2; g.OW = PER ? 2 * g.Kw : 2 * g.Kw - LT + 2;
            g.per_d0 = 0; g.head_off = -1;
            if ((int64_t)g.Kh * g.Kw >= (1LL << 28)) return WL_ERR_UNSUPPORTED;
            g.rbytes = g.Kw * SZ;
            if (g.rbytes % 4 != 0 || ((int64_t)g.Kh * g.rbytes) % 4 != 0 || (uintptr_t)yh[j] % 4 != 0) return WL_ERR_UNSUPPORTED;
#ifndef WL_IROWS_R0
#define WL_IROWS_R0 8
#endif
            g.dma_rows = j == 0 ? WL_IROWS_R0 : 8; g.dma_shift = j == 0 && WL_IROWS_R0 == 16 ? 4 : 3;
            if (PER) {
                g.per_d0 = wl_align_up(WARM * SZ, 16);
                g.rbytes = wl_align_up(g.per_d0 + g.Kw * SZ, 16);
                g.per_grp = 1;
#ifndef WL_IROWS_PER_GRP
#define WL_IROWS_PER_GRP 8
#endif
                if ((g.Kw * SZ) % 16 == 0)
                    while (g.per_grp < WL_IROWS_PER_GRP && 2 * g.per_grp * g.rbytes <= WL_IROWS_CHUNK) g.per_grp *= 2;
                while (g.dma_rows < 4 * g.per_grp) { g.dma_rows *= 2; ++g.dma_shift; }
            } else g.per_grp = 1;
            while (!PER && (g.dma_rows < wl_cdiv(WL_IROWS_CHUNK, g.rbytes) + 4 || (g.dma_rows * g.rbytes) % 16)) { g.dma_rows *= 2; ++g.dma_shift; }
            g.cpr = wl_cdiv(g.dma_rows * g.rbytes, WL_IROWS_CHUNK);
            g.nwaves = wl_cdiv(wl_cdiv(g.OW, 2), 64);
            compute_waves += g.nwaves;
            sh = g.OH; sw = g.OW;
        }
        if (ll_rs != a.g[nlev - 1].Kw || (ll_ps * SZ) % 4 != 0 || (uintptr_t)yl % 4 != 0) return WL_ERR_UNSUPPORTED;
        if (PER && (yl_h != a.g[nlev - 1].Kh || yl_w != a.g[nlev - 1].Kw)) return WL_ERR_UNSUPPORTED;
        if ((int64_t)a.g[0].OH * a.g[0].OW >= (1LL << 28)) return WL_ERR_UNSUPPORTED;
    }
    struct Ld { int level, s0, ns; } ld[8];
    int nld = 0;
    const bool one_loader = nlev == 1 && compute_waves <= 2;
    if (one_loader) ld[nld++] = Ld{0, 0, 4};
    else if (nlev == 1) for (int s = 0; s < 4; ++s) ld[nld++] = Ld{0, s, 1};
    else {
#ifndef WL_IROWS_NARROW_ML
#define WL_IROWS_NARROW_ML 2
#endif
        const bool narrow_ml = WL_IROWS_NARROW_ML && strips != 2 && compute_waves <= nlev + WL_IROWS_NARROW_ML - 1 &&
                               WL_IROWS_WAVES / (compute_waves + nlev) > WL_IROWS_WAVES / (compute_waves + nlev + 2);
        if (narrow_ml) ld[nld++] = Ld{0, 1, 3};
        else for (int s = 1; s < 4; ++s) ld[nld++] = Ld{0, s, 1};
        for (int j = 1; j < nlev; ++j) ld[nld++] = Ld{j, j == nlev - 1 ? 0 : 1, j == nlev - 1 ? 4 : 3};
    }
    if (compute_waves + nld > WL_IROWS_WAVES) return WL_ERR_UNSUPPORTED;
    for (int l = 0; l < nld; ++l) {
        if (PER) {
            const int rowb = a.g[ld[l].level].Kw * SZ;
            const int per_row = a.g[ld[l].level].per_grp > 1 ? ld[l].ns : ld[l].ns * (wl_cdiv(rowb & ~15, WL_IROWS_CHUNK) + ((rowb & 15) ? 1 : 0));
            if (WL_IROWS_MAX_VM / per_row - 1 < 4) return WL_ERR_UNSUPPORTED;
        } else if (2 * wl_cdiv(a.g[ld[l].level].rbytes, WL_IROWS_CHUNK) + 2 > WL_IROWS_MAX_VM / ld[l].ns - 1) return WL_ERR_UNSUPPORTED;
    }
    int pp_waves = WL_IROWS_WAVES / (compute_waves + nld);
#ifdef WL_IROWS_PP_MAX
    if (pp_waves > WL_IROWS_PP_MAX) pp_waves = WL_IROWS_PP_MAX;
#endif
    for (int t = 0; t < 3; ++t) {
        a.seg[t].own_lo = a.seg[t].own_hi = a.seg[t].nhb = 0;
        for (int j = 0; j < WL_IROWS_MAXLEV; ++j) a.seg[t].f0[j] = a.seg[t].fend[j] = 0;
    }
    const int OH0 = a.g[0].OH;
    int M = (OH0 / 2) & ~1;
    if (PER) M &= ~((2 << nlev) - 1);
    bool can_split = M >= 2 && M + 2 <= OH0;
    for (int t = 0; t < 3; ++t)
        for (int j = 0; j < WL_IROWS_MAXLEV; ++j) a.seg[t].rho[j] = 0;
    for (int t = 0; t < (can_split ? 3 : 1); ++t) {
        WlIRowsSeg& sg = a.seg[t];
        sg.own_lo = t == 2 ? M : 0;
        sg.own_hi = t == 1 ? M : OH0;
        if (PER) {
            const int len = sg.own_hi - sg.own_lo;
            for (int j = 0; j < nlev; ++j) sg.rho[j] = (sg.own_lo / 2) >> j;
            sg.own_lo = 0; sg.own_hi = len;
            sg.f0[0] = 0;
            sg.fend[0] = len / 2 + WARM;
            for (int j = 1; j < nlev; ++j) {
                sg.f0[j] = 0;
                int rows = sg.fend[j - 1];
                if (rows > a.g[j - 1].Kh) rows = a.g[j - 1].Kh;
                sg.fend[j] = (rows + 1) / 2 + WARM;
            }
            continue;
        }
        sg.f0[0] = sg.own_lo / 2;
        sg.fend[0] = (sg.own_hi + 1) / 2 + WARM;
        if (sg.fend[0] > a.g[0].Kh) sg.fend[0] = a.g[0].Kh;
        for (int j = 1; j < nlev; ++j) {
            sg.f0[j] = sg.f0[j - 1] / 2;
            sg.fend[j] = (sg.fend[j - 1] - 1) / 2 + WARM + 1;
            if (sg.fend[j] > a.g[j].Kh) sg.fend[j] = a.g[j].Kh;
        }
    }
    int off = 0;
    for (int rr = 4;; rr *= 2) {
        off = 0;
        for (int j = 0; j < nlev; ++j) {
            WlIRowsLevel& g = a.g[j];
            if (j + 1 < nlev) {
                int cols = g.Kw;
                if (2 * wl_cdiv(a.g[j + 1].OW, 2) > cols) cols = 2 * wl_cdiv(a.g[j + 1].OW, 2);
                if (PER) cols += WARM;
                g.ll_rows = rr; g.ll_pitch = wl_align_up(cols * SZ, 16);
            } else { g.ll_rows = g.dma_rows; g.ll_pitch = g.rbytes; }
            for (int s = 0; s < 4; ++s) {
                g.src_off[s] = off;
                off += s == 0 ? g.ll_rows * g.ll_pitch : wl_align_up(g.dma_rows * g.rbytes, 16);
                if (PER && s == 0 && j + 1 < nlev) { g.head_off = off; off += (WARM > 0 ? WARM : 1) * g.ll_pitch; }
            }
        }
        bool ok = true;
        for (int t = 0; t < (can_split ? 3 : 1); ++t) {
            const int rc = wl_irows_plan_segment<T>(a, a.seg[t], LT);
            if (rc) { if (t == 0) return rc; can_split = false; break; }
            WlIRowsArgs<T> b = a;
            for (int j = 0; j < nlev; ++j) b.g[j].ll_rows = 1 << 20;
            wl_irows_plan_segment<T>(b, b.seg[t], LT);
            if (a.seg[t].nhb > b.seg[t].nhb + 2) ok = false;
        }
        if (ok || nlev == 1) break;
        if (rr >= 64) return WL_ERR_UNSUPPORTED;
    }
    for (int j = nlev; j < WL_IROWS_MAXLEV; ++j) { a.g[j] = a.g[nlev - 1]; a.g[j].nwaves = 0; a.yh[j] = nullptr; }
    if (off > 80 * 1024) return WL_ERR_UNSUPPORTED;
    int pp = pp_waves;
    a.lds_plane = wl_align_up(off, 16);
    while (pp > 1 && (pp * a.lds_plane > 80 * 1024 || (planes + pp - 1) / pp < (int64_t)wl_num_cus())) --pp;
    if (strips == 2) pp = 1;
    bool pack_cut = false;
    if (strips == 0 && can_split && pp == 1 && pp_waves > 1) {
        const int64_t slots = 2 * (int64_t)wl_num_cus();
        const int64_t r1 = (planes + slots - 1) / slots;
        const bool halves = r1 == 1 && r1 * slots - planes > 0 && planes > wl_num_cus();
        const int64_t cost_now = halves ? ((2 * planes + slots - 1) / slots) * (int64_t)(OH0 / 4 + LT / 2 + 8) : r1 * (int64_t)(OH0 / 2 + 8);
        const int p2 = wl_rows_pack_and_cut(planes, pp_waves, a.lds_plane, OH0 / 2, LT / 2, cost_now, slots);
        if (p2) { pp = p2; pack_cut = true; }
    }
    a.pp = pp;
    if (pp > 1) off = pp * a.lds_plane;
    a.lds_bytes = off;
    {
        int load[4] = {0, 0, 0, 0}, cnt[4] = {0, 0, 0, 0};
        const int cap[4] = {(WL_IROWS_WAVES + 3) / 4, (WL_IROWS_WAVES + 2) / 4, (WL_IROWS_WAVES + 1) / 4, WL_IROWS_WAVES / 4};
        for (int w = 0; w < WL_IROWS_WAVES; ++w) { a.role_level[w] = -2; a.role_arg[w] = 0; a.role_sub[w] = 0; }
        int sub = 0;
        auto place = [&](int level, int arg, int cost) {
            int best = -1;
            for (int b = 0; b < 4; ++b)
                if (cnt[b] < cap[b] && (best < 0 || load[b] < load[best])) best = b;
            const int w = best + 4 * cnt[best];
            a.role_level[w] = (signed char)level; a.role_arg[w] = (short)arg; a.role_sub[w] = (signed char)sub;
            load[best] += cost; ++cnt[best];
        };
        for (sub = 0; sub < pp; ++sub)
            for (int j = 0; j < nlev; ++j)
                for (int c = 0; c < a.g[j].nwaves; ++c) place(j, 64 * c, 16 >> j);
        for (sub = 0; sub < pp; ++sub)
            for (int l = 0; l < nld; ++l) place(-1, ld[l].level * 16 + ld[l].s0 * 4 + (ld[l].ns - 1), ld[l].level == 0 ? 3 : 2);
    }
    if (strips == 2 && !can_split) return WL_ERR_UNSUPPORTED;
    const int64_t units = (planes + pp - 1) / pp;
    int64_t ncut = 0;
    if (can_split && strips == 2) ncut = planes;
    else if (pack_cut) ncut = units;
    else if (can_split && strips == 0 && pp == 1) {
        const int64_t cus = wl_num_cus(), slots = 2 * cus;
        const int64_t rounds = (planes + slots - 1) / slots;
        ncut = rounds * slots - planes;
        if (ncut > planes) ncut = planes;
        if (rounds > 1 && ncut * 4 > planes) ncut = 0;
        if (rounds == 1 && ncut > 0) ncut = planes;
        if (planes <= cus) ncut = cus - planes < planes ? cus - planes : planes;
    }
    a.nwhole = (int)(units - ncut);
    a.yl = (const T*)yl; a.ll_ps = ll_ps;
    for (int j = 0; j < nlev; ++j) a.yh[j] = (const T*)yh[j];
    a.y = (T*)r.y;
    a.g_w_lo = (const float*)r.taps.w_lo; a.g_w_hi = (const float*)r.taps.w_hi;
    a.g_h_lo = (const float*)r.taps.h_lo; a.g_h_hi = (const float*)r.taps.h_hi;
    a.NC = planes;
    a.guard = guard; a.lat = lat;
    if (what == 1) return 0;
    return what == 2 ? wl_launch_armed<K>(a, units + ncut, (size_t)off, r.stream) : wl_launch<K>(a, units + ncut, (size_t)off, r.stream);
}

template <typename T, int LT, int PER = 0>
static int wl_sfb_rows_pick(const WlSfbPyrReq& r) {
    if constexpr (LT >= WL_IROWS_LAT_MIN) {
        if ((r.hints & 3) == 3 && r.scratch)
            return wl_lattice_launch<LT>([&](int guard, int what) { return wl_sfb_rows_launch<T, LT, 0, PER>(r, r.scratch, guard, what); },
                                         [&](int guard, int what) { return wl_sfb_rows_launch<T, LT, 1, PER>(r, r.scratch, guard, what); },
                                         r.taps, 1, 1, sizeof(T), r.scratch, r.tstate, 3, r.stream);
    }
    if constexpr (LT > 12) return WL_ERR_UNSUPPORTED;
    else return wl_sfb_rows_launch<T, LT, 0, PER>(r);
}

template <typename T>
static int wl_sfb_rows_dispatch(const WlSfbPyrReq& r) {
#define WL_CASE(LT_) case LT_: return r.mode == 2 ? wl_sfb_rows_pick<T, LT_, 1>(r) : wl_sfb_rows_pick<T, LT_, 0>(r)
    switch (r.L) {
        WL_CASE(2); WL_CASE(4); WL_CASE(6); WL_CASE(8); WL_CASE(10); WL_CASE(12); WL_CASE(14); WL_CASE(16); WL_CASE(18); WL_CASE(20);
        default: return WL_ERR_UNSUPPORTED;
    }
#undef WL_CASE
}

extern "C" int wl_dwt2d_synthesis_fused_ex(const void* yl, int64_t yl_plane_stride, int yl_row_stride, int yl_h, int yl_w,
                                           const void* const* yh, const int* Kh, const int* Kw, void* y, int dtype,
                                           int64_t planes, int nlev, const void* g_w_lo, const void* g_w_hi,
                                           const void* g_h_lo, const void* g_h_hi, int L, int mode, int strips,
                                           void* tap_scratch, int* tap_state, void* stream) {
    if (wl_mode_to_ext(mode) < 0) return WL_ERR_MODE;
    if (planes < 0 || yl_h < 1 || yl_w < 1) return WL_ERR_SHAPE;
    if (L < 1 || L > WL_MAX_TAPS) return WL_ERR_TAPS;
    if (strips > 15) return WL_ERR_UNSUPPORTED;
    const int hints = strips < 0 ? 0 : ((strips & 4) ? 1 : 0) | ((strips & 8) ? 2 : 0);
    if (!tap_scratch) tap_state = nullptr;
    if (strips >= 0) strips &= 3;
    if (strips < 0 || strips > 2) return WL_ERR_UNSUPPORTED;
    if (strips == 0 && 8 * planes < 3 * wl_num_cus()) return WL_ERR_UNSUPPORTED;
    if (planes == 0) return 0;
    const WlSfbPyrReq r = {yl, yl_plane_stride, yl_row_stride, yl_h, yl_w, yh, Kh, Kw, y, planes, nlev,
                           {g_w_lo, g_w_hi, g_h_lo, g_h_hi}, L, mode, strips, hints, (float*)tap_scratch, tap_state, stream};
    WL_DISPATCH_FLOAT(dtype, return wl_sfb_rows_dispatch<T>(r));
}

extern "C" int wl_dwt2d_synthesis_fused(const void* yl, int64_t yl_plane_stride, int yl_row_stride, int yl_h, int yl_w,
                                        const void* const* yh, const int* Kh, const int* Kw, void* y, int dtype,
                                        int64_t planes, int nlev, const void* g_w_lo, const void* g_w_hi,
                                        const void* g_h_lo, const void* g_h_hi, int L, int mode, int strips, void* stream) {
    return wl_dwt2d_synthesis_fused_ex(yl, yl_plane_stride, yl_row_stride, yl_h, yl_w, yh, Kh, Kw, y, dtype, planes, nlev,
                                       g_w_lo, g_w_hi, g_h_lo, g_h_hi, L, mode, strips, nullptr, nullptr, stream);
}
#endif
```

pytorch_wavelets_amd/ops.py:

```python
import contextlib
import ctypes
import threading
import torch

from . import _lib

_DTYPES = {torch.float32: 0, torch.float16: 1, torch.float64: 2, torch.bfloat16: 3}
_TEST_BACKEND = None


def _backend():
    return _TEST_BACKEND if _TEST_BACKEND is not None else _lib.get()


def _check_tensor(t, name):
    if t.dtype not in _DTYPES:
        raise TypeError('%s: unsupported dtype %s (float16/bfloat16/float32/float64)' % (name, t.dtype))
    if not t.is_cuda and _TEST_BACKEND is None:
        raise RuntimeError('%s is on %s: pytorch_wavelets_amd runs on MI355X only (HIP kernels, '
                           'no CPU fallback). Move the module and its input to a cuda device.'
                           % (name, t.device))


class _NoGuard(object):
    def __enter__(self):
        return self

    def __exit__(self, *exc):
        return False


_NOGUARD = _NoGuard()


def _device_of(t):
    return torch.cuda.device(t.device) if t.is_cuda else _NOGUARD


def _same_device(*ts):
    dev = None
    for t in ts:
        if t is None:
            continue
        if dev is None:
            dev = t.device
        elif t.device != dev:
            raise RuntimeError('pytorch_wavelets_amd: tensors on different devices (%s, %s)' % (dev, t.device))


def _call(name, ref, *args):
    with _device_of(ref):
        return getattr(_backend(), name)(*args)


def _stream(t):
    return torch.cuda.current_stream(t.device).cuda_stream if t.is_cuda else None


def _taps(h, ref):
    acc = torch.float64 if ref.dtype == torch.float64 else torch.float32
    return h.detach().reshape(-1).to(device=ref.device, dtype=acc).contiguous()


def coeff_len(n, L, mode):
    return (n + 1) // 2 if mode == 2 else (n + L - 1) // 2


def synth_len(K, L, mode, crop=None):
    n = 2 * K if mode == 2 else 2 * K - L + 2
    return n if crop is None else min(n, crop)


def _synth_hw(Kh, Kw, Lh, Lw, mode, out_hw=None):
    crop_h, crop_w = (out_hw[0], out_hw[1]) if out_hw is not None else (None, None)
    return synth_len(Kh, Lh, mode, crop_h), synth_len(Kw, Lw, mode, crop_w)


def _outer_inner(shape, dim):
    outer = inner = 1
    for v in shape[:dim]:
        outer *= v
    for v in shape[dim + 1:]:
        inner *= v
    return outer, inner


def _new_pyramid(x, nlev, L, mode, axes):
    lead, size = tuple(x.shape[:-axes]), tuple(x.shape[-axes:])
    band = (3,) if axes == 2 else ()
    yh = []
    for _ in range(nlev):
        size = tuple(coeff_len(n, L, mode) for n in size)
        yh.append(torch.empty(lead + band + size, dtype=x.dtype, device=x.device))
    yl = torch.empty(lead + size, dtype=x.dtype, device=x.device)
    return yh, yl, (ctypes.c_void_p * nlev)(*[t.data_ptr() for t in yh])


def _plane_strides(t):
    N, C, H, W = t.shape
    s0, s1, s2, s3 = t.stride()
    if W > 1 and s3 != 1:
        return None
    rs = s2 if H > 1 else W
    if rs < W:
        return None
    if C > 1:
        ps = s1
        if N > 1 and s0 != C * ps:
            return None
    elif N > 1:
        ps = s0
    else:
        ps = H * rs
    if ps < 0:
        return None
    return ps, rs


def _planes(t):
    st = None if t.numel() == 0 else _plane_strides(t)
    if st is None:
        t = t.contiguous()
        st = (t.shape[2] * t.shape[3], t.shape[3])
    return t, st[0], st[1]


def _ll_pitch(kw, itemsize):
    q = 128 // itemsize
    return (kw + q - 1) // q * q


def afb2d(x, h_w_lo, h_w_hi, h_h_lo, h_h_hi, mode, pad_ll=False):
    _check_tensor(x, 'x')
    N, C, H, W = x.shape
    x, x_ps, x_rs = _planes(x)
    hwl, hwh, hhl, hhh = (_taps(h, x) for h in (h_w_lo, h_w_hi, h_h_lo, h_h_hi))
    Lw, Lh = hwl.numel(), hhl.numel()
    Kh, Kw = coeff_len(H, Lh, mode), coeff_len(W, Lw, mode)
    if pad_ll:
        ll = torch.empty((N, C, Kh, _ll_pitch(Kw, x.element_size())), dtype=x.dtype, device=x.device)[..., :Kw]
    else:
        ll = torch.empty((N, C, Kh, Kw), dtype=x.dtype, device=x.device)
    highs = torch.empty((N, C, 3, Kh, Kw), dtype=x.dtype, device=x.device)
    rc = _call('wl_dwt2d_analysis_strided', x, x.data_ptr(), x_ps, x_rs, ll.data_ptr(), ll.stride(1),
                                              ll.stride(2), highs.data_ptr(), _DTYPES[x.dtype], N * C, H, W,
                                              hwl.data_ptr(), hwh.data_ptr(), Lw, hhl.data_ptr(), hhh.data_ptr(), Lh,
                                              mode, _stream(x))
    _lib.check(rc, 'wl_dwt2d_analysis_strided')
    return ll, highs


def sfb2d(ll, highs, g_w_lo, g_w_hi, g_h_lo, g_h_hi, mode, out_hw=None):
    _check_tensor(ll, 'll')
    N, C, Kh, Kw = ll.shape
    ll, ll_ps, ll_rs = _planes(ll)
    if highs is not None:
        if highs.dtype != ll.dtype:
            highs = highs.to(ll.dtype)
        highs = highs.contiguous()
        if tuple(highs.shape) != (N, C, 3, Kh, Kw):
            raise ValueError('highs %s does not match ll %s' % (tuple(highs.shape), tuple(ll.shape)))
        _same_device(ll, highs)
    gwl, gwh, ghl, ghh = (_taps(g, ll) for g in (g_w_lo, g_w_hi, g_h_lo, g_h_hi))
    Lw, Lh = gwl.numel(), ghl.numel()
    OH, OW = _synth_hw(Kh, Kw, Lh, Lw, mode, out_hw)
    y = torch.empty((N, C, OH, OW), dtype=ll.dtype, device=ll.device)
    rc = _call('wl_dwt2d_synthesis', ll, ll.data_ptr(), ll_ps, ll_rs,
                                       None if highs is None else highs.data_ptr(), y.data_ptr(),
                                       _DTYPES[ll.dtype], N * C, Kh, Kw, OH, OW, gwl.data_ptr(),
                                       gwh.data_ptr(), Lw, ghl.data_ptr(), ghh.data_ptr(), Lh, mode,
                                       _stream(ll))
    _lib.check(rc, 'wl_dwt2d_synthesis')
    return y


_CU_COUNT = {}
_HINTS = threading.local()


class TapVerdict(object):

    def __init__(self, fn):
        self.fn = fn
        self.key = None
        self.val = False

    def __call__(self, *bufs):
        try:
            key = tuple((b.data_ptr(), b._version, b.dtype, b.device, tuple(b.shape)) for b in bufs)
        except (RuntimeError, AttributeError):
            try:
                key = tuple((b.data_ptr(), -1, b.dtype, b.device, tuple(b.shape)) for b in bufs)
            except (RuntimeError, AttributeError):
                return False
        if key != self.key:
            self.val = bool(self.fn(*bufs))
            self.key = key
        return self.val


def is_qmf_pair(lo, hi):
    a, b = lo.detach().reshape(-1).double().cpu(), hi.detach().reshape(-1).double().cpu()
    if a.numel() != b.numel() or a.numel() % 2 or a.numel() == 0:
        return False
    sign = torch.tensor([1.0, -1.0], dtype=torch.float64).repeat(a.numel() // 2)
    return bool(torch.equal(b, sign * a.flip(0)))


def is_symmetric_taps(h):
    a = h.detach().reshape(-1).double().cpu()
    return a.numel() > 0 and bool(torch.equal(a, a.flip(0)))


@contextlib.contextmanager
def qmf_hint(flag):
    prev = getattr(_HINTS, 'qmf', False), getattr(_HINTS, 'tapcache', None)
    _HINTS.qmf = bool(flag)
    _HINTS.tapcache = {} if flag else None
    try:
        yield
    finally:
        _HINTS.qmf, _HINTS.tapcache = prev


def _hinted_taps(bufs, ref, L, syn):
    cache = getattr(_HINTS, 'tapcache', None)
    key = (tuple((b.data_ptr(), b.dtype) for b in bufs), ref.device, ref.dtype, L, bool(syn))
    ent = cache.get(key) if cache is not None else None
    if ent is None:
        taps = tuple(_taps(b, ref) for b in bufs)
        scratch = _new_tap_scratch(ref.device) if L >= min(ROWS_LATTICE_MIN, IROWS_LATTICE_MIN) and (STRIP_LATTICE or ROWS_LATTICE) else None
        ent = [taps, scratch, ctypes.c_int(0)]
        if cache is not None:
            cache[key] = ent
    return ent


def _new_tap_scratch(device):
    return torch.empty(TAP_SCRATCH_FLOATS, dtype=torch.float32, device=device)


def _launch_taps(bufs, ref, L, syn, hinted):
    if not hinted:
        return tuple(_taps(b, ref) for b in bufs), None, ctypes.c_int(0)
    taps, scratch, tstate = _hinted_taps(bufs, ref, L, syn)
    return taps, None if scratch is None else scratch.data_ptr(), tstate


def _fused_hint_bits(same, qmf):
    return (4 if same else 0) | (8 if qmf else 0)


def _strip_policy_bits(force, qmf):
    return (1 if force else 0) | (2 if qmf else 0)


def current_hints():
    return bool(getattr(_HINTS, 'qmf', False)), bool(getattr(_HINTS, 'same', False))


@contextlib.contextmanager
def hints(qmf, same):
    with qmf_hint(qmf), same_banks_hint(same):
        yield


def banks_equal(lo_a, hi_a, lo_b, hi_b):
    f = lambda t: t.detach().reshape(-1).double().cpu()
    return (lo_a.numel() == lo_b.numel() and hi_a.numel() == hi_b.numel() and lo_a.numel() > 0
            and bool(torch.equal(f(lo_a), f(lo_b))) and bool(torch.equal(f(hi_a), f(hi_b))))


@contextlib.contextmanager
def same_banks_hint(flag):
    prev = getattr(_HINTS, 'same', False)
    _HINTS.same = bool(flag)
    try:
        yield
    finally:
        _HINTS.same = prev


STREAM_FORCE = False
FUSED_STRIPS = 0
_FUSED_DECLINED = set()
_FUSED_DECLINED_MAX = 4096


def _remember_decline(key):
    be = _backend()
    if be.wl_get_option(b'generic_only') or be.wl_get_option(b'no_stream') or be.wl_get_option(b'scat_stream'):
        return
    if len(_FUSED_DECLINED) >= _FUSED_DECLINED_MAX:
        _FUSED_DECLINED.clear()
    _FUSED_DECLINED.add(key)


def _declined(key, name, ref, *args, memo=True):
    rc = _call(name, ref, *args)
    if rc == _lib.WL_ERR_UNSUPPORTED:
        if memo:
            _remember_decline(key)
        return True
    _lib.check(rc, name)
    return False


def set_option(name, value):
    _FUSED_DECLINED.clear()
    rc = _backend().wl_set_option(name.encode() if isinstance(name, str) else name, int(value))
    _lib.check(rc, 'wl_set_option')


def _num_cus(device):
    if device.type != 'cuda':
        return 2
    idx = device.index if device.index is not None else torch.cuda.current_device()
    if idx not in _CU_COUNT:
        _CU_COUNT[idx] = torch.cuda.get_device_properties(idx).multi_processor_count
    return _CU_COUNT[idx]


def afb2d_fused(x, h_w_lo, h_w_hi, h_h_lo, h_h_hi, mode, nlev, strips=None, whole=True):
    _check_tensor(x, 'x')
    if strips is None:
        strips = FUSED_STRIPS
    N, C, H, W = x.shape
    L = h_w_lo.numel()
    qmf, same = current_hints()
    lattice = (same and qmf and ROWS_LATTICE and L in (8, 10, 12, 14, 16, 18, 20) and L >= ROWS_LATTICE_MIN
               and (L > 12 or x.numel() >= LATTICE_MIN_ELEMS or (mode == 2 and L == 12)))
    if L == 20 and h_w_lo.element_size() == 2 and strips == 0:
        return None
    if (x.dtype == torch.float64 or nlev < 1 or nlev > 3 or h_h_lo.numel() != L or L % 2 or (L > 12 and not lattice)
            or (nlev > 1 and mode not in (0, 1, 2, 4)) or x.numel() == 0 or (mode == 2 and not ROWS_PER and (nlev > 1 or L % 4 == 0))
            or (strips == 0 and 8 * N * C < 3 * _num_cus(x.device)) or strips > 2):
        return None
    es = x.element_size()
    if mode == 2 and es == 2 and L % 4 == 0 and L >= 12:
        return None
    if (W * es > 2048 and not ROWS_3KIB) or (W * es >= 2048 and nlev < 2 and not whole):
        return None
    x, x_ps, x_rs = _planes(x)
    if (x_rs * es) % 16 or (x_ps * es) % 16 or x.data_ptr() % 16 or (W * es + 15) // 16 * 16 > x_rs * es:
        return None
    key = ('afb', x.device, x.dtype, N * C, H, W, x_ps, x_rs, L, mode, nlev, strips, lattice)
    if key in _FUSED_DECLINED:
        return None
    (hwl, hwh, hhl, hhh), scratch, tstate = _launch_taps((h_w_lo, h_w_hi, h_h_lo, h_h_hi), x, L, False, lattice)
    yh, yl, ptrs = _new_pyramid(x, nlev, L, mode, 2)
    if _declined(key, 'wl_dwt2d_analysis_fused_ex', x, x.data_ptr(), x_ps, x_rs, yl.data_ptr(), ptrs, _DTYPES[x.dtype], N * C, H, W, nlev,
                 hwl.data_ptr(), hwh.data_ptr(), hhl.data_ptr(), hhh.data_ptr(), L, mode, strips | _fused_hint_bits(same, qmf),
                 scratch, ctypes.byref(tstate), _stream(x)):
        return None
    return yl, yh


SMALL_PLANES = True


def afb2d_small(x, h_w_lo, h_w_hi, h_h_lo, h_h_hi, mode, nlev):
    _check_tensor(x, 'x')
    N, C, H, W = x.shape
    L = h_w_lo.numel()
    if (not SMALL_PLANES or FUSED_STRIPS or STREAM_FORCE or x.dtype == torch.float64 or nlev < 1 or nlev > 4 or h_h_lo.numel() != L or L > 20 or x.numel() == 0
            or H * W > 5184 or mode not in _MODE_TO_EXT):
        return None
    key = ('afbsm', x.device, x.dtype, N * C, H, W, L, mode, nlev)
    if key in _FUSED_DECLINED:
        return None
    x = x.contiguous()
    hwl, hwh, hhl, hhh = (_taps(h, x) for h in (h_w_lo, h_w_hi, h_h_lo, h_h_hi))
    yh, yl, ptrs = _new_pyramid(x, nlev, L, mode, 2)
    if _declined(key, 'wl_dwt2d_analysis_small', x, x.data_ptr(), yl.data_ptr(), ptrs, _DTYPES[x.dtype], N * C, H, W, nlev,
                 hwl.data_ptr(), hwh.data_ptr(), hhl.data_ptr(), hhh.data_ptr(), L, mode, _stream(x)):
        return None
    return yl, yh


def sfb2d_small(yl, yh, g_w_lo, g_w_hi, g_h_lo, g_h_hi, mode):
    _check_tensor(yl, 'yl')
    nlev = len(yh)
    N, C, h, w = yl.shape
    L = g_w_lo.numel()
    if (not SMALL_PLANES or FUSED_STRIPS or STREAM_FORCE or yl.dtype == torch.float64 or nlev < 1 or nlev > 4
            or g_h_lo.numel() != L or L % 2 or L > 20 or yl.numel() == 0 or mode not in _MODE_TO_EXT
            or any(t is None or t.dim() != 5 or t.dtype != yl.dtype or t.shape[:3] != (N, C, 3) or t.numel() == 0 for t in yh)):
        return None
    OH, OW = _synth_hw(yh[0].shape[3], yh[0].shape[4], L, L, mode)
    if OH < 1 or OW < 1 or OH * OW > 5184:
        return None
    key = ('sfbsm', yl.device, yl.dtype, N * C, h, w, tuple(tuple(t.shape[3:]) for t in yh), L, mode)
    if key in _FUSED_DECLINED:
        return None
    yl = yl.contiguous()
    yh = [t.contiguous() for t in yh]
    for t in yh:
        _same_device(yl, t)
    gwl, gwh, ghl, ghh = (_taps(g, yl) for g in (g_w_lo, g_w_hi, g_h_lo, g_h_hi))
    y = torch.empty((N, C, OH, OW), dtype=yl.dtype, device=yl.device)
    ptrs = (ctypes.c_void_p * nlev)(*[t.data_ptr() for t in yh])
    khs = (ctypes.c_int * nlev)(*[t.shape[3] for t in yh])
    kws = (ctypes.c_int * nlev)(*[t.shape[4] for t in yh])
    if _declined(key, 'wl_dwt2d_synthesis_small', yl, yl.data_ptr(), h, w, ptrs, khs, kws, y.data_ptr(), _DTYPES[yl.dtype], N * C, nlev,
                 gwl.data_ptr(), gwh.data_ptr(), ghl.data_ptr(), ghh.data_ptr(), L, mode, _stream(yl)):
        return None
    return y


def sfb2d_fused(yl, yh, g_w_lo, g_w_hi, g_h_lo, g_h_hi, mode, strips=None):
    _check_tensor(yl, 'yl')
    if strips is None:
        strips = FUSED_STRIPS
    nlev = len(yh)
    N, C, h, w = yl.shape
    L = g_w_lo.numel()
    es = yl.element_size()
    qmf, same = current_hints()
    lattice = (same and qmf and ROWS_LATTICE and L in (8, 10, 12, 14, 16, 18, 20) and L >= IROWS_LATTICE_MIN
               and (L > 12 or (nlev >= 1 and yh[0] is not None and yh[0].dim() == 5
                               and 4 * yh[0].shape[3] * yh[0].shape[4] * N * C >= (LATTICE_MIN_ELEMS if nlev == 1 else min(LATTICE_MIN_ELEMS, LATTICE_MIN_ELEMS_ML)))))
    if es == 2 and L > IROWS_F16_MAXL and strips == 0:
        return None
    per = mode == 2
    if per and not IROWS_PER:
        return None
    if per and strips == 0 and IROWS_PER_POLICY and nlev >= 1 and yh[0] is not None and yh[0].dim() == 5:
        ow0 = 2 * yh[0].shape[4]
        if (L > 12 or N * C < _num_cus(yl.device) or (es == 4 and ow0 < 320)
                or (es == 2 and (L > 4 or not 384 <= ow0 <= 512))):
            return None
    if (yl.dtype == torch.float64 or nlev < 1 or nlev > 3 or g_h_lo.numel() != L or L % 2 or (L > 12 and not lattice)
            or yl.numel() == 0 or (strips == 0 and 8 * N * C < 3 * _num_cus(yl.device)) or strips > 2
            or any(t is None or t.dim() != 5 or t.dtype != yl.dtype or t.shape[:3] != (N, C, 3) or t.numel() == 0
                   or (t.shape[4] * es) % 4 or (t.shape[3] * t.shape[4] * es) % 4 for t in yh)):
        return None
    sh, sw = h, w
    for t in reversed(yh):
        kh, kw = t.shape[3], t.shape[4]
        if not (kh <= sh <= kh + 1 and kw <= sw <= kw + 1) or kh < L // 2 or kw < L // 2 or (per and (sh, sw) != (kh, kw)):
            return None
        sh, sw = _synth_hw(kh, kw, L, L, mode)
    kh, kw = yh[-1].shape[3], yh[-1].shape[4]
    if (h, w) != (kh, kw):
        yl = yl[..., :kh, :kw]
    st = _plane_strides(yl)
    if st is None or st[1] != kw or (st[0] * es) % 4:
        yl = yl.contiguous()
        st = (kh * kw, kw)
    yl_ps, yl_rs = st
    yh = [t.contiguous() for t in yh]
    for t in yh:
        _same_device(yl, t)
    key = ('sfb', yl.device, yl.dtype, N * C, kh, kw, tuple(tuple(t.shape[3:]) for t in yh), L, mode, strips, lattice)
    if key in _FUSED_DECLINED or yl.data_ptr() % 4 or any(t.data_ptr() % 4 for t in yh):
        return None
    (gwl, gwh, ghl, ghh), scratch, tstate = _launch_taps((g_w_lo, g_w_hi, g_h_lo, g_h_hi), yl, L, True, lattice)
    y = torch.empty((N, C, sh, sw), dtype=yl.dtype, device=yl.device)
    ptrs = (ctypes.c_void_p * nlev)(*[t.data_ptr() for t in yh])
    khs = (ctypes.c_int * nlev)(*[t.shape[3] for t in yh])
    kws = (ctypes.c_int * nlev)(*[t.shape[4] for t in yh])
    if _declined(key, 'wl_dwt2d_synthesis_fused_ex', yl, yl.data_ptr(), yl_ps, yl_rs, kh, kw, ptrs, khs, kws,
                 y.data_ptr(), _DTYPES[yl.dtype], N * C, nlev, gwl.data_ptr(), gwh.data_ptr(), ghl.data_ptr(),
                 ghh.data_ptr(), L, mode, strips | _fused_hint_bits(same, qmf), scratch, ctypes.byref(tstate), _stream(yl)):
        return None
    return y


STRIP_MINW = 128
TAP_SCRATCH_FLOATS = 16
STRIP_LATTICE = True
ROWS_LATTICE = True
ROWS_LATTICE_MIN = 10
LATTICE_MIN_ELEMS = 40000000
LATTICE_MIN_ELEMS_ML = 16000000
IROWS_LATTICE_MIN = 8


IROWS_F16_MAXL = 8
IROWS_PER_POLICY = True
IROWS_PER = True
ROWS_PER = True
ROWS_3KIB = True
PAD_ODD_LL = True


def afb2d_stream(x, h_w_lo, h_w_hi, h_h_lo, h_h_hi, mode, force=False, pad_ll=False):
    _check_tensor(x, 'x')
    N, C, H, W = x.shape
    L = h_w_lo.numel()
    es = x.element_size()
    if (x.dtype == torch.float64 or h_h_lo.numel() != L or L % 2 or L > 20 or W < 2 * L or H < 2 or x.numel() == 0
            or (mode in (2, 6) and W % 4) or (mode == 2 and (H + (H & 1) < L - 1 or W + (W & 1) < L - 1))):
        return None
    if not force and W < STRIP_MINW:
        return None
    x, x_ps, x_rs = _planes(x)
    qmf = current_hints()[0]
    key = ('afbs', x.device, x.dtype, N * C, H, W, x_ps, x_rs, L, mode, bool(force), qmf, bool(pad_ll))
    if key in _FUSED_DECLINED:
        return None
    (hwl, hwh, hhl, hhh), scratch, tstate = _launch_taps((h_w_lo, h_w_hi, h_h_lo, h_h_hi), x, L, False, qmf)
    Kh, Kw = coeff_len(H, L, mode), coeff_len(W, L, mode)
    q = 16 // es
    Kp = (Kw + q - 1) // q * q if pad_ll else Kw
    ll = torch.empty((N, C, Kh, Kp), dtype=x.dtype, device=x.device)
    if Kp != Kw:
        ll = ll[..., :Kw]
    highs = torch.empty((N, C, 3, Kh, Kw), dtype=x.dtype, device=x.device)
    if _declined(key, 'wl_dwt2d_analysis_stream_ex', x, x.data_ptr(), x_ps, x_rs, ll.data_ptr(), Kh * Kp, Kp, highs.data_ptr(),
                 _DTYPES[x.dtype], N * C, H, W, hwl.data_ptr(), hwh.data_ptr(), hhl.data_ptr(), hhh.data_ptr(), L, mode,
                 _strip_policy_bits(force, qmf), scratch, ctypes.byref(tstate), _stream(x)):
        return None
    return ll, highs


def sfb2d_stream(ll, highs, g_w_lo, g_w_hi, g_h_lo, g_h_hi, mode, out_hw=None, force=False):
    _check_tensor(ll, 'll')
    if highs is None or ll.dtype == torch.float64:
        return None
    N, C, Kh, Kw = ll.shape
    L = g_w_lo.numel()
    es = ll.element_size()
    if (g_h_lo.numel() != L or L % 2 or L > 20 or (mode == 2 and Kw % 4) or Kw < L or Kh < L // 2 or ll.numel() == 0
            or tuple(highs.shape) != (N, C, 3, Kh, Kw) or highs.dtype != ll.dtype
            or (mode == 2 and (2 * Kh < L - 2 or 2 * Kw < L - 2))):
        return None
    OH, OW = _synth_hw(Kh, Kw, L, L, mode, out_hw)
    if not force and (OW < STRIP_MINW or OW % 4):
        return None
    ll, ll_ps, ll_rs = _planes(ll)
    highs = highs.contiguous()
    _same_device(ll, highs)
    qmf = current_hints()[0]
    key = ('sfbs', ll.device, ll.dtype, N * C, Kh, Kw, ll_ps, ll_rs, OH, OW, L, mode, bool(force), qmf)
    if key in _FUSED_DECLINED:
        return None
    (gwl, gwh, ghl, ghh), scratch, tstate = _launch_taps((g_w_lo, g_w_hi, g_h_lo, g_h_hi), ll, L, True, qmf)
    y = torch.empty((N, C, OH, OW), dtype=ll.dtype, device=ll.device)
    if _declined(key, 'wl_dwt2d_synthesis_stream_ex', ll, ll.data_ptr(), ll_ps, ll_rs, highs.data_ptr(), y.data_ptr(), _DTYPES[ll.dtype],
                 N * C, Kh, Kw, OH, OW, gwl.data_ptr(), gwh.data_ptr(), ghl.data_ptr(), ghh.data_ptr(), L, mode,
                 _strip_policy_bits(force, qmf), scratch, ctypes.byref(tstate), _stream(ll)):
        return None
    return y


def sfb2d_best(ll, highs, g_w_lo, g_w_hi, g_h_lo, g_h_hi, mode, out_hw=None):
    res = sfb2d_stream(ll, highs, g_w_lo, g_w_hi, g_h_lo, g_h_hi, mode, out_hw=out_hw, force=STREAM_FORCE)
    return res if res is not None else sfb2d(ll, highs, g_w_lo, g_w_hi, g_h_lo, g_h_hi, mode, out_hw=out_hw)


def afb2d_best(x, h_w_lo, h_w_hi, h_h_lo, h_h_hi, mode, pad_ll=False, more_levels=False):
    if x.dim() == 4:
        res = afb2d_small(x, h_w_lo, h_w_hi, h_h_lo, h_h_hi, mode, 1)
        if res is not None:
            return res[0], res[1][0]
    res = afb2d_stream(x, h_w_lo, h_w_hi, h_h_lo, h_h_hi, mode, force=STREAM_FORCE, pad_ll=more_levels and PAD_ODD_LL)
    return res if res is not None else afb2d(x, h_w_lo, h_w_hi, h_h_lo, h_h_hi, mode, pad_ll=pad_ll)


def afb2d_nonsep(x, filts, mode):
    _check_tensor(x, 'x')
    if filts.dim() != 4 or filts.shape[0] != 4 or filts.shape[1] != 1:
        raise ValueError('filts must be a (4, 1, Ly, Lx) tensor, got %s' % (tuple(filts.shape),))
    x = x.contiguous()
    N, C, H, W = x.shape
    Ly, Lx = filts.shape[2], filts.shape[3]
    f = _taps(filts, x)
    y = torch.empty((N, 4 * C, coeff_len(H, Ly, mode), coeff_len(W, Lx, mode)), dtype=x.dtype, device=x.device)
    if x.numel():
        rc = _call('wl_dwt2d_analysis_nonsep', x, x.data_ptr(), y.data_ptr(), _DTYPES[x.dtype], N * C, H, W,
                   f.data_ptr(), Ly, Lx, mode, _stream(x))
        _lib.check(rc, 'wl_dwt2d_analysis_nonsep')
    return y


def sfb2d_nonsep(coeffs, filts, mode, out_hw=None):
    _check_tensor(coeffs, 'coeffs')
    if filts.dim() != 4 or filts.shape[0] != 4 or filts.shape[1] != 1:
        raise ValueError('filts must be a (4, 1, Ly, Lx) tensor, got %s' % (tuple(filts.shape),))
    if coeffs.dim() == 5:
        if coeffs.shape[2] != 4:
            raise ValueError('coeffs must be (N, C, 4, H, W), got %s' % (tuple(coeffs.shape),))
        N, C, _, Kh, Kw = coeffs.shape
    else:
        if coeffs.dim() != 4 or coeffs.shape[1] % 4:
            raise ValueError('coeffs must be (N, C, 4, H, W) or (N, 4C, H, W), got %s' % (tuple(coeffs.shape),))
        N, C, Kh, Kw = coeffs.shape[0], coeffs.shape[1] // 4, coeffs.shape[2], coeffs.shape[3]
    coeffs = coeffs.contiguous()
    Ly, Lx = filts.shape[2], filts.shape[3]
    g = _taps(filts, coeffs)
    OH, OW = _synth_hw(Kh, Kw, Ly, Lx, mode, out_hw)
    y = torch.empty((N, C, OH, OW), dtype=coeffs.dtype, device=coeffs.device)
    if coeffs.numel():
        rc = _call('wl_dwt2d_synthesis_nonsep', coeffs, coeffs.data_ptr(), y.data_ptr(), _DTYPES[coeffs.dtype], N * C,
                   Kh, Kw, OH, OW, g.data_ptr(), Ly, Lx, mode, _stream(coeffs))
        _lib.check(rc, 'wl_dwt2d_synthesis_nonsep')
    return y


def afb2d_nonsep_bwd(dy, filts, mode, in_hw):
    _check_tensor(dy, 'dy')
    dy = dy.contiguous()
    H, W = in_hw
    N, C4 = dy.shape[:2]
    Ly, Lx = filts.shape[2], filts.shape[3]
    if tuple(dy.shape[2:]) != (coeff_len(H, Ly, mode), coeff_len(W, Lx, mode)) or C4 % 4:
        raise ValueError('afb2d_nonsep_bwd: dy %s does not belong to a %dx%d input' % (tuple(dy.shape), H, W))
    f = _taps(filts, dy)
    dx = torch.empty((N, C4 // 4, H, W), dtype=dy.dtype, device=dy.device)
    if dx.numel():
        rc = _call('wl_dwt2d_analysis_nonsep_bwd', dy, dy.data_ptr(), dx.data_ptr(), _DTYPES[dy.dtype], N * (C4 // 4), H, W,
                   f.data_ptr(), Ly, Lx, mode, _stream(dy))
        _lib.check(rc, 'wl_dwt2d_analysis_nonsep_bwd')
    return dx


def sfb2d_nonsep_bwd(dy, filts, mode, coeff_shape):
    _check_tensor(dy, 'dy')
    dy = dy.contiguous()
    N, C = dy.shape[:2]
    Kh, Kw = coeff_shape[-2], coeff_shape[-1]
    Ly, Lx = filts.shape[2], filts.shape[3]
    g = _taps(filts, dy)
    dc = torch.empty((N, C, 4, Kh, Kw), dtype=dy.dtype, device=dy.device)
    if dc.numel():
        rc = _call('wl_dwt2d_synthesis_nonsep_bwd', dy, dy.data_ptr(), dc.data_ptr(), _DTYPES[dy.dtype], N * C, Kh, Kw,
                   g.data_ptr(), Ly, Lx, mode, _stream(dy))
        _lib.check(rc, 'wl_dwt2d_synthesis_nonsep_bwd')
    return dc.reshape(coeff_shape)


EXT_ZERO, EXT_SYM, EXT_REFL, EXT_PERIODIC, EXT_PER, EXT_REPLICATE, EXT_PER_FOLD1 = 0, 1, 2, 3, 4, 5, 6
_MODE_TO_EXT = {0: EXT_ZERO, 1: EXT_SYM, 2: EXT_PER, 4: EXT_REFL, 6: EXT_PERIODIC}


def corr1d(x, dim, h0, h1, K, start, step, tap_step=1, ext=EXT_SYM, taps=None, out=None, out_offset=0, out_stride=1,
           ny=None):
    _check_tensor(x, 'x')
    x = x.contiguous()
    dim = dim % x.dim()
    n = x.shape[dim]
    outer, inner = _outer_inner(x.shape, dim)
    t0 = _taps(h0, x)
    t1 = None if h1 is None else _taps(h1, x)
    off, ts, nt = taps if taps is not None else (0, 1, t0.numel())
    if ny is None:
        ny = out_offset + out_stride * K
    shape = list(x.shape)
    shape[dim] = ny
    if out is None:
        alloc = torch.empty if (out_stride == 1 and out_offset == 0 and ny == K) else torch.zeros
        out = (alloc(shape, dtype=x.dtype, device=x.device),
               None if h1 is None else alloc(shape, dtype=x.dtype, device=x.device))
    y0, y1 = out
    if x.numel() and K:
        rc = _call('wl_corr1d', x, x.data_ptr(), y0.data_ptr(), None if y1 is None else y1.data_ptr(), _DTYPES[x.dtype],
                   outer, n, inner, ny * inner, K, t0.data_ptr(), None if t1 is None else t1.data_ptr(), off, ts, nt,
                   start, step, tap_step, ext, out_offset, out_stride, _stream(x))
        _lib.check(rc, 'wl_corr1d')
    return (y0, y1) if h1 is not None else y0


def afb1d(x, h0, h1, mode, dim):
    n, L = x.shape[dim], h0.numel()
    K = coeff_len(n, L, mode)
    if mode == 2:
        if n + (n & 1) < L - 1:
            return corr1d(x, dim, h0, h1, K, 1 - L, 2, 1, EXT_PER_FOLD1)
        base = L // 2 - L + 1
    else:
        base = -((2 * (K - 1) - n + L) // 2)
    return corr1d(x, dim, h0, h1, K, base, 2, 1, _MODE_TO_EXT[mode])


def afb1d_fused(x, h0, h1, mode, J):
    _check_tensor(x, 'x')
    L = h0.numel()
    n = x.shape[-1]
    if (x.dtype == torch.float64 or J < 1 or J > 4 or L % 2 or L > 20 or h1.numel() != L or x.numel() == 0 or n < L
            or mode not in _MODE_TO_EXT):
        return None
    x = x.contiguous()
    rows = x.numel() // n
    key = ('afb1d', x.device, x.dtype, rows, n, L, mode, J)
    if key in _FUSED_DECLINED:
        return None
    t0, t1 = _taps(h0, x), _taps(h1, x)
    his, lo, ptrs = _new_pyramid(x, J, L, mode, 1)
    if _declined(key, 'wl_dwt1d_analysis_fused', x, x.data_ptr(), lo.data_ptr(), ptrs, _DTYPES[x.dtype], rows, n, J, t0.data_ptr(),
                 t1.data_ptr(), L, mode, _stream(x)):
        return None
    return lo, his


def swt2d_level(x, h_w_lo, h_w_hi, h_h_lo, h_h_hi, dilation, ext):
    _check_tensor(x, 'x')
    N, C, H, W = x.shape
    Lw, Lh = h_w_lo.numel(), h_h_lo.numel()
    if h_w_hi.numel() != Lw or h_h_hi.numel() != Lh or x.numel() == 0:
        return None
    st = _plane_strides(x)
    if st is None or st[1] != W:
        x = x.contiguous()
        st = (H * W, W)
    key = ('swt2d', x.device, x.dtype, N * C, H, W, st[0], Lw, Lh, dilation, ext)
    if key in _FUSED_DECLINED:
        return None
    taps = [_taps(h, x) for h in (h_w_lo, h_w_hi, h_h_lo, h_h_hi)]
    y = torch.empty((N, 4 * C, H, W), dtype=x.dtype, device=x.device)
    if _declined(key, 'wl_swt2d_level', x, x.data_ptr(), st[0], y.data_ptr(), _DTYPES[x.dtype], N * C, H, W,
                 taps[0].data_ptr(), taps[1].data_ptr(), taps[2].data_ptr(), taps[3].data_ptr(), Lw, Lh, dilation, ext, _stream(x)):
        return None
    return y


def iswt2d_level(y, h_w_lo, h_w_hi, h_h_lo, h_h_hi, dilation, ext, scale=1.0, ll=None, ll_mode=0):
    ref = y if y is not None else ll
    _check_tensor(ref, 'y')
    if (ll is None) != (ll_mode == 0) or (y is None and ll_mode != 1):
        raise ValueError('iswt2d_level: ll_mode %d does not go with the tensors given' % ll_mode)
    if y is not None:
        N, C4, H, W = y.shape
        if C4 % 4:
            raise ValueError('iswt2d_level: y has %d channels, not four sub-bands per input channel' % C4)
        C = C4 // 4
        y = y.contiguous()
    else:
        N, C, H, W = ll.shape
    ll_ps = 0
    if ll is not None:
        _same_device(y, ll)
        if tuple(ll.shape) != (N, C, H, W) or ll.dtype != ref.dtype:
            raise ValueError('iswt2d_level: ll is %s %s, expected %s %s' % (tuple(ll.shape), ll.dtype, (N, C, H, W), ref.dtype))
        st = None if ll.numel() == 0 else _plane_strides(ll)
        if st is None or st[1] != W:
            ll = ll.contiguous()
            st = (H * W, W)
        ll_ps = st[0]
    Lw, Lh = h_w_lo.numel(), h_h_lo.numel()
    if h_w_hi.numel() != Lw or h_h_hi.numel() != Lh or ref.numel() == 0:
        return None
    key = ('iswt2d', ref.device, ref.dtype, N * C, H, W, y is None, ll_ps, ll_mode, Lw, Lh, dilation, ext)
    if key in _FUSED_DECLINED:
        return None
    taps = [_taps(h, ref) for h in (h_w_lo, h_w_hi, h_h_lo, h_h_hi)]
    x = torch.empty((N, C, H, W), dtype=ref.dtype, device=ref.device)
    if _declined(key, 'wl_iswt2d_level', ref, None if y is None else y.data_ptr(), 4 * H * W, None if ll is None else ll.data_ptr(), ll_ps,
                 ll_mode, x.data_ptr(), _DTYPES[ref.dtype], N * C, H, W, taps[0].data_ptr(), taps[1].data_ptr(), taps[2].data_ptr(),
                 taps[3].data_ptr(), Lw, Lh, dilation, ext, float(scale), _stream(ref)):
        return None
    return x


def _outer_stride(t, dim):
    shape, st = t.shape, t.stride()
    inner = 1
    for k in range(t.dim() - 1, dim - 1, -1):
        if shape[k] > 1 and st[k] != inner:
            return None
        inner *= shape[k]
    os_, span = None, 1
    for k in range(dim - 1, -1, -1):
        if shape[k] == 1:
            continue
        if os_ is None:
            os_ = st[k]
            if os_ < inner:
                return None
        elif st[k] != os_ * span:
            return None
        span *= shape[k]
    return inner if os_ is None else os_


def _with_outer_stride(t, dim):
    if t is None:
        return None, 0
    os_ = _outer_stride(t, dim) if t.numel() else None
    if os_ is None:
        t = t.contiguous()
        os_ = _outer_stride(t, dim) if t.numel() else 0
    return t, os_


def corr1d_adj(y0, y1, dim, h0, h1, n, start, tap_step=1, ext=EXT_SYM, scale=1.0):
    _check_tensor(y0, 'y0')
    if ext not in (EXT_ZERO, EXT_SYM, EXT_REFL, EXT_PERIODIC, EXT_REPLICATE):
        raise ValueError('corr1d_adj: extension %r has no transpose here' % (ext,))
    if (y1 is None) != (h1 is None):
        raise ValueError('corr1d_adj: y1 and h1 go together')
    dim = dim % y0.dim()
    if y1 is not None:
        _same_device(y0, y1)
        if y1.shape != y0.shape or y1.dtype != y0.dtype:
            raise ValueError('corr1d_adj: y0 is %s %s, y1 is %s %s' % (tuple(y0.shape), y0.dtype, tuple(y1.shape), y1.dtype))
    y0, os0 = _with_outer_stride(y0, dim)
    y1, os1 = _with_outer_stride(y1, dim)
    K = y0.shape[dim]
    outer, inner = _outer_inner(y0.shape, dim)
    t0 = _taps(h0, y0)
    t1 = None if h1 is None else _taps(h1, y0)
    shape = list(y0.shape)
    shape[dim] = n
    dx = torch.empty(shape, dtype=y0.dtype, device=y0.device)
    if dx.numel():
        rc = _call('wl_corr1d_adj', y0, y0.data_ptr(), os0, None if y1 is None else y1.data_ptr(), os1, dx.data_ptr(),
                   _DTYPES[y0.dtype], outer, n, inner, K, t0.data_ptr(), None if t1 is None else t1.data_ptr(), t0.numel(), start,
                   tap_step, ext, float(scale), _stream(y0))
        _lib.check(rc, 'wl_corr1d_adj')
    return dx


def sfb1d_fused(lo, his, g0, g1, mode, out_len=None):
    _check_tensor(lo, 'lo')
    J, L = len(his), g0.numel()
    if (lo.dtype == torch.float64 or J < 1 or J > 4 or L % 2 or L > 20 or g1.numel() != L or lo.numel() == 0 or mode == 2
            or mode not in _MODE_TO_EXT or all(h is None for h in his)):
        return None
    lens = []
    for j, h in enumerate(his):
        if h is None:
            return None
        if h.dtype != lo.dtype or h.shape[:-1] != lo.shape[:-1]:
            return None
        lens.append(h.shape[-1])
    full = synth_len(lens[0], L, mode)
    if out_len is None:
        out_len = full
    if out_len < 1 or out_len > full:
        return None
    key = ('sfb1d', lo.device, lo.dtype, lo.numel() // lo.shape[-1], lo.shape[-1], tuple(lens), L, mode, out_len)
    if key in _FUSED_DECLINED:
        return None
    lo = lo.contiguous()
    his = [h.contiguous() for h in his]
    for h in his:
        _same_device(lo, h)
    rows = lo.numel() // lo.shape[-1]
    t0, t1 = _taps(g0, lo), _taps(g1, lo)
    y = torch.empty(lo.shape[:-1] + (out_len,), dtype=lo.dtype, device=lo.device)
    ptrs = (ctypes.c_void_p * J)(*[h.data_ptr() for h in his])
    ns = (ctypes.c_int * J)(*lens)
    if _declined(key, 'wl_dwt1d_synthesis_fused', lo, lo.data_ptr(), lo.shape[-1], ptrs, ns, y.data_ptr(), out_len, _DTYPES[lo.dtype], rows, J,
                 t0.data_ptr(), t1.data_ptr(), L, mode, _stream(lo)):
        return None
    return y


def sfb1d(lo, hi, g0, g1, mode, dim, out_len=None):
    _check_tensor(lo, 'lo')
    lo = lo.contiguous()
    dim = dim % lo.dim()
    K, L = lo.shape[dim], g0.numel()
    if hi is not None:
        hi = hi.to(lo.dtype).contiguous()
        if hi.shape != lo.shape:
            raise ValueError('lo %s and hi %s differ in shape' % (tuple(lo.shape), tuple(hi.shape)))
        _same_device(lo, hi)
    ny = synth_len(K, L, mode, out_len)
    outer, inner = _outer_inner(lo.shape, dim)
    shape = list(lo.shape)
    shape[dim] = ny
    y = torch.empty(shape, dtype=lo.dtype, device=lo.device)
    t0, t1 = _taps(g0, lo), _taps(g1, lo)
    if y.numel():
        rc = _call('wl_synth1d', lo, lo.data_ptr(), None if hi is None else hi.data_ptr(), y.data_ptr(), _DTYPES[lo.dtype],
                   outer, K, inner, ny, t0.data_ptr(), t1.data_ptr(), L, mode, _stream(lo))
        _lib.check(rc, 'wl_synth1d')
    return y


def dtcwt_fwd1(x, h0, h1, mode, skip_hps=False):
    _check_tensor(x, 'x')
    x = x.contiguous()
    N, C, H, W = x.shape
    t0, t1 = _taps(h0, x), _taps(h1, x)
    He, We = H + (H & 1), W + (W & 1)
    ll = torch.empty((N, C, He, We), dtype=x.dtype, device=x.device)
    highs = None if skip_hps else torch.empty((N, C, 6, He // 2, We // 2, 2), dtype=x.dtype, device=x.device)
    rc = _call('wl_dtcwt_fwd_level1', x, x.data_ptr(), ll.data_ptr(), None if skip_hps else highs.data_ptr(),
                                        _DTYPES[x.dtype], N * C, H, W, t0.data_ptr(), t0.numel(), t1.data_ptr(),
                                        t1.numel(), mode, _stream(x))
    _lib.check(rc, 'wl_dtcwt_fwd_level1')
    return ll, highs


def dtcwt_fwd1_rot(x, h0, h1, h2, symmetric, scat=False, magbias=0.0):
    _check_tensor(x, 'x')
    if x.dim() != 4 or x.numel() == 0:
        return None
    N, C, H, W = x.shape
    key = ('dtrot', x.device, x.dtype, N, C, H, W, h0.numel(), h1.numel(), h2.numel(), bool(symmetric), bool(scat))
    if key in _FUSED_DECLINED:
        return None
    x = x.contiguous()
    t0, t1, t2 = _taps(h0, x), _taps(h1, x), _taps(h2, x)
    h2_, w2_ = H // 2, W // 2
    if scat:
        ll = im = None
        re = torch.empty((N, 7, C, h2_, w2_), dtype=x.dtype, device=x.device)
    else:
        ll = torch.empty((N, C, H, W), dtype=x.dtype, device=x.device)
        re = torch.empty((N, 6, C, h2_, w2_), dtype=x.dtype, device=x.device)
        im = torch.empty_like(re)
    if _declined(key, 'wl_dtcwt_fwd_level1_rot', x, x.data_ptr(), None if ll is None else ll.data_ptr(), re.data_ptr(),
                 None if im is None else im.data_ptr(), _DTYPES[x.dtype], N, C, H, W, t0.data_ptr(), t0.numel(), t1.data_ptr(),
                 t1.numel(), t2.data_ptr(), t2.numel(), 1 if symmetric else 0, 1 if scat else 0, float(magbias), _stream(x)):
        return None
    return re if scat else (ll, re, im)


def dtcwt_fwd12(x, h0o, h1o, h0a, h0b, h1a, h1b, mode, force=False):
    _check_tensor(x, 'x')
    N, C, H, W = x.shape
    if mode != 1 or H % 4 or W % 4 or x.dtype not in (torch.float32, torch.float16, torch.bfloat16):
        return None
    force = force or STREAM_FORCE
    key = ('dt12', x.device, x.dtype, N * C, H, W, h0o.numel(), h1o.numel(), h0a.numel(), mode)
    if not force and key in _FUSED_DECLINED:
        return None
    x = x.contiguous()
    t0, t1 = _taps(h0o, x), _taps(h1o, x)
    ta, tb, tc, td = (_taps(h, x) for h in (h0a, h0b, h1a, h1b))
    highs1 = torch.empty((N, C, 6, H // 2, W // 2, 2), dtype=x.dtype, device=x.device)
    ll2 = torch.empty((N, C, H // 2, W // 2), dtype=x.dtype, device=x.device)
    highs2 = torch.empty((N, C, 6, H // 4, W // 4, 2), dtype=x.dtype, device=x.device)
    if _declined(key, 'wl_dtcwt_fwd_level12', x, x.data_ptr(), highs1.data_ptr(), ll2.data_ptr(), highs2.data_ptr(),
                 _DTYPES[x.dtype], N * C, H, W, t0.data_ptr(), t0.numel(), t1.data_ptr(), t1.numel(), ta.data_ptr(),
                 tb.data_ptr(), tc.data_ptr(), td.data_ptr(), ta.numel(), mode, 1 if force else 0, _stream(x), memo=not force):
        return None
    return highs1, ll2, highs2


def dtcwt_fwd2(x, h0a, h0b, h1a, h1b, skip_hps=False):
    _check_tensor(x, 'x')
    x = x.contiguous()
    N, C, H, W = x.shape
    ta, tb, tc, td = (_taps(h, x) for h in (h0a, h0b, h1a, h1b))
    He, We = H + (2 if H % 4 else 0), W + (2 if W % 4 else 0)
    ll = torch.empty((N, C, He // 2, We // 2), dtype=x.dtype, device=x.device)
    highs = None if skip_hps else torch.empty((N, C, 6, He // 4, We // 4, 2), dtype=x.dtype, device=x.device)
    rc = _call('wl_dtcwt_fwd_level2', x, x.data_ptr(), ll.data_ptr(), None if skip_hps else highs.data_ptr(),
                                        _DTYPES[x.dtype], N * C, H, W, ta.data_ptr(), tb.data_ptr(), tc.data_ptr(),
                                        td.data_ptr(), ta.numel(), _stream(x))
    _lib.check(rc, 'wl_dtcwt_fwd_level2')
    return ll, highs


def dtcwt_inv1(ll, highs, g0, g1, mode):
    ref = ll if ll is not None else highs
    _check_tensor(ref, 'coeffs')
    if highs is not None:
        highs = highs.contiguous()
        N, C = highs.shape[:2]
        H, W = 2 * highs.shape[3], 2 * highs.shape[4]
    else:
        N, C, H, W = ll.shape
    ps = rs = 0
    if ll is not None:
        if tuple(ll.shape) != (N, C, H, W):
            raise ValueError('lowpass %s does not match the highpass size %s' % (tuple(ll.shape), (N, C, H, W)))
        _same_device(ll, highs)
        ll, ps, rs = _planes(ll)
    t0, t1 = _taps(g0, ref), _taps(g1, ref)
    y = torch.empty((N, C, H, W), dtype=ref.dtype, device=ref.device)
    rc = _call('wl_dtcwt_inv_level1', ref, None if ll is None else ll.data_ptr(), ps, rs,
                                        None if highs is None else highs.data_ptr(), y.data_ptr(),
                                        _DTYPES[ref.dtype], N * C, H, W, t0.data_ptr(), t0.numel(), t1.data_ptr(),
                                        t1.numel(), mode, _stream(ref))
    _lib.check(rc, 'wl_dtcwt_inv_level1')
    return y


def dtcwt_inv2(ll, highs, g0a, g0b, g1a, g1b):
    ref = ll if ll is not None else highs
    _check_tensor(ref, 'coeffs')
    if highs is not None:
        highs = highs.contiguous()
        N, C = highs.shape[:2]
        h, w = 2 * highs.shape[3], 2 * highs.shape[4]
    else:
        N, C, h, w = ll.shape
    ps = rs = 0
    if ll is not None:
        if tuple(ll.shape) != (N, C, h, w):
            raise ValueError('lowpass %s does not match the highpass size %s' % (tuple(ll.shape), (N, C, h, w)))
        _same_device(ll, highs)
        ll, ps, rs = _planes(ll)
    ta, tb, tc, td = (_taps(g, ref) for g in (g0a, g0b, g1a, g1b))
    y = torch.empty((N, C, 2 * h, 2 * w), dtype=ref.dtype, device=ref.device)
    rc = _call('wl_dtcwt_inv_level2', ref, None if ll is None else ll.data_ptr(), ps, rs,
                                        None if highs is None else highs.data_ptr(), y.data_ptr(),
                                        _DTYPES[ref.dtype], N * C, h, w, ta.data_ptr(), tb.data_ptr(), tc.data_ptr(),
                                        td.data_ptr(), ta.numel(), _stream(ref))
    _lib.check(rc, 'wl_dtcwt_inv_level2')
    return y


def dtcwt_inv21(ll2, highs2, highs1, g0o, g1o, g0a, g0b, g1a, g1b, mode, force=False):
    _check_tensor(ll2, 'll2')
    if highs2 is None or highs1 is None or highs1.dim() != 6 or highs2.dim() != 6:
        return None
    N, C, h, w = ll2.shape
    if (mode != 1 or h % 2 or w % 2 or ll2.dtype not in (torch.float32, torch.float16, torch.bfloat16) or highs1.dtype != ll2.dtype
            or highs2.dtype != ll2.dtype or tuple(highs2.shape) != (N, C, 6, h // 2, w // 2, 2)
            or tuple(highs1.shape) != (N, C, 6, h, w, 2) or ll2.numel() == 0):
        return None
    force = force or STREAM_FORCE
    _same_device(ll2, highs2, highs1)
    ll2, ps, rs = _planes(ll2)
    key = ('dti21', ll2.device, ll2.dtype, N * C, h, w, ps, rs, g0o.numel(), g1o.numel(), g0a.numel(), mode)
    if not force and key in _FUSED_DECLINED:
        return None
    highs2, highs1 = highs2.contiguous(), highs1.contiguous()
    t0, t1 = _taps(g0o, ll2), _taps(g1o, ll2)
    ta, tb, tc, td = (_taps(g, ll2) for g in (g0a, g0b, g1a, g1b))
    y = torch.empty((N, C, 2 * h, 2 * w), dtype=ll2.dtype, device=ll2.device)
    if _declined(key, 'wl_dtcwt_inv_level21', ll2, ll2.data_ptr(), ps, rs, highs2.data_ptr(), highs1.data_ptr(), y.data_ptr(),
                 _DTYPES[ll2.dtype], N * C, 2 * h, 2 * w, t0.data_ptr(), t0.numel(), t1.data_ptr(), t1.numel(), ta.data_ptr(),
                 tb.data_ptr(), tc.data_ptr(), td.data_ptr(), ta.numel(), mode, 1 if force else 0, _stream(ll2), memo=not force):
        return None
    return y


def scat_fwd1(x, h0, h1, mode, magbias, combine_colour, save, want_ll=False):
    _check_tensor(x, 'x')
    x = x.contiguous()
    N, C, H, W = x.shape
    t0, t1 = _taps(h0, x), _taps(h1, x)
    h2, w2 = (H + (H & 1)) // 2, (W + (W & 1)) // 2
    z = torch.empty((N, 9, h2, w2) if combine_colour else (N, 7, C, h2, w2), dtype=x.dtype, device=x.device)
    dx = dy = ll = None
    if save:
        dx = torch.empty((N, 6, C, h2, w2), dtype=x.dtype, device=x.device)
        dy = torch.empty_like(dx)
    if want_ll:
        ll = torch.empty((N, C, 2 * h2, 2 * w2), dtype=x.dtype, device=x.device)
    rc = _call('wl_scat_fwd_level1', x, x.data_ptr(), z.data_ptr(), None if dx is None else dx.data_ptr(),
               None if dy is None else dy.data_ptr(), None if ll is None else ll.data_ptr(), _DTYPES[x.dtype], N, C, H, W,
               t0.data_ptr(), t0.numel(), t1.data_ptr(), t1.numel(), mode, float(magbias),
               1 if combine_colour else 0, _stream(x))
    _lib.check(rc, 'wl_scat_fwd_level1')
    return (z, dx, dy, ll) if want_ll else (z, dx, dy)


def scat_fwd1_into(x, z, z_bs, z_ll_off, z_mag_off, h0, h1, mode, magbias, ll=None):
    _check_tensor(x, 'x')
    x = x.contiguous()
    N, C, H, W = x.shape
    q = (H // 2) * (W // 2)
    assert H % 2 == 0 and W % 2 == 0 and z.is_contiguous() and z.dtype == x.dtype and z.device == x.device
    last = (N - 1) * z_bs + max(z_ll_off + C * q, z_mag_off + 6 * C * q)
    assert N == 0 or (min(z_bs, z_mag_off) >= 0 and last <= z.numel()), 'entries outside z'
    t0, t1 = _taps(h0, x), _taps(h1, x)
    rc = _call('wl_scat_fwd_level1_into', x, x.data_ptr(), z.data_ptr(), z_bs, z_ll_off, z_mag_off,
               None if ll is None else ll.data_ptr(), _DTYPES[x.dtype], N, C, H, W, t0.data_ptr(), t0.numel(), t1.data_ptr(),
               t1.numel(), mode, float(magbias), _stream(x))
    _lib.check(rc, 'wl_scat_fwd_level1_into')


def scat_fwd2_into(x, z, z_bs, z_ll_off, z_mag_off, h0a, h0b, h1a, h1b, magbias):
    _check_tensor(x, 'x')
    x = x.contiguous()
    N, C, H, W = x.shape
    q = (H // 4) * (W // 4)
    assert z.is_contiguous() and z.dtype == x.dtype and z.device == x.device
    last = (N - 1) * z_bs + max(z_ll_off + C * q, z_mag_off + 6 * C * q)
    assert N == 0 or (min(z_bs, z_ll_off, z_mag_off) >= 0 and last <= z.numel()), 'entries outside z'
    key = ('scat2', x.device, x.dtype, N, C, H, W, int(h0a.numel()), z_bs, z_ll_off, z_mag_off)
    if H % 4 or W % 4 or key in _FUSED_DECLINED:
        return False
    ta, tb, tc, td = (_taps(h, x) for h in (h0a, h0b, h1a, h1b))
    return not _declined(key, 'wl_scat_fwd_level2_into', x, x.data_ptr(), z.data_ptr(), z_bs, z_ll_off, z_mag_off, _DTYPES[x.dtype], N, C, H, W,
                         ta.data_ptr(), tb.data_ptr(), tc.data_ptr(), td.data_ptr(), ta.numel(), float(magbias), _stream(x))


def scat_bwd1(dz, drdx, drdy, h0, h1, mode, combine_colour):
    _check_tensor(dz, 'dz')
    dz = dz.contiguous()
    N, _, C, h2, w2 = drdx.shape
    if drdy.shape != drdx.shape or drdx.dtype != dz.dtype or drdy.dtype != dz.dtype:
        raise ValueError('scat_bwd1: drdx %s / drdy %s / dz dtype mismatch' % (tuple(drdx.shape), tuple(drdy.shape)))
    want = (N, 9, h2, w2) if combine_colour else (N, 7, C, h2, w2)
    if tuple(dz.shape) != want:
        raise ValueError('scat_bwd1: dz %s, expected %s' % (tuple(dz.shape), want))
    _same_device(dz, drdx, drdy)
    drdx, drdy = drdx.contiguous(), drdy.contiguous()
    t0, t1 = _taps(h0, dz), _taps(h1, dz)
    dx = torch.empty((N, C, 2 * h2, 2 * w2), dtype=dz.dtype, device=dz.device)
    if _declined(None, 'wl_scat_bwd_level1', dz, dz.data_ptr(), drdx.data_ptr(), drdy.data_ptr(), dx.data_ptr(), _DTYPES[dz.dtype],
                 N, C, 2 * h2, 2 * w2, t0.data_ptr(), t0.numel(), t1.data_ptr(), t1.numel(), mode,
                 1 if combine_colour else 0, _stream(dz), memo=False):
        return None
    return dx
```

Measured before the change: 300,800 Mpixels/s.

## Precompute lattice factorisation on host and self-verify in one synthesis launch for 8 taps

For 8-tap filters, the lattice factor of the synthesis filters is now computed on the host, cached by tensor identity, and passed by value into the rows synthesis kernel. A new LAT=2 kernel form checks on the device that the hint reproduces the taps and picks the lattice or direct body per wave, which removes the separate factorisation or guard launch and its scratch round trip. In exchange it adds a CPU copy of the taps on a cache miss and a per-block verification cost, and it raises the default lattice minimum for the old path to 10 taps.

```diff
diff --git a/include/wavelets_hip.h b/include/wavelets_hip.h
--- a/include/wavelets_hip.h
+++ b/include/wavelets_hip.h
@@ -61,6 +61,12 @@
                                 int64_t planes, int nlev, const void* g_w_lo, const void* g_w_hi,
                                 const void* g_h_lo, const void* g_h_hi, int L, int mode, int strips, void* tap_scratch,
                                 int* tap_state, void* stream);
+int wl_dwt2d_synthesis_fused_hint(const void* yl, int64_t yl_plane_stride, int yl_row_stride, int yl_h, int yl_w,
+                                  const void* const* yh, const int* Kh, const int* Kw, void* y, int dtype,
+                                  int64_t planes, int nlev, const void* g_w_lo, const void* g_w_hi,
+                                  const void* g_h_lo, const void* g_h_hi, int L, int mode, int strips, void* tap_scratch,
+                                  int* tap_state, const float* lattice_hint, void* lattice_verdict, void* stream);
+int wl_lattice_factor_host(const float* lo, const float* hi, int L, int syn, double tol, float* out);
 
 int wl_dwt2d_analysis_nonsep(const void* x, void* y, int dtype, int64_t planes, int H, int W, const void* f,
                              int Ly, int Lx, int mode, void* stream);
diff --git a/pytorch_wavelets_amd/_capi.py b/pytorch_wavelets_amd/_capi.py
--- a/pytorch_wavelets_amd/_capi.py
+++ b/pytorch_wavelets_amd/_capi.py
@@ -21,6 +21,9 @@
     'wl_dwt2d_analysis_fused_ex': (I, [P, L, I, P, C.POINTER(P), I, L, I, I, I, P, P, P, P, I, I, I, P, C.POINTER(I), P]),
     'wl_dwt2d_synthesis_fused': (I, [P, L, I, I, I, C.POINTER(P), C.POINTER(I), C.POINTER(I), P, I, L, I, P, P, P, P, I, I, I, P]),
     'wl_dwt2d_synthesis_fused_ex': (I, [P, L, I, I, I, C.POINTER(P), C.POINTER(I), C.POINTER(I), P, I, L, I, P, P, P, P, I, I, I, P, C.POINTER(I), P]),
+    'wl_dwt2d_synthesis_fused_hint': (I, [P, L, I, I, I, C.POINTER(P), C.POINTER(I), C.POINTER(I), P, I, L, I, P, P, P, P, I, I, I, P, C.POINTER(I),
+                                           C.POINTER(C.c_float), P, P]),
+    'wl_lattice_factor_host': (I, [C.POINTER(C.c_float), C.POINTER(C.c_float), I, I, C.c_double, C.POINTER(C.c_float)]),
     'wl_dwt2d_analysis_stream': (I, [P, L, I, P, L, I, P, I, L, I, I, P, P, P, P, I, I, I, P]),
     'wl_dwt2d_analysis_stream_ex': (I, [P, L, I, P, L, I, P, I, L, I, I, P, P, P, P, I, I, I, P, C.POINTER(I), P]),
     'wl_dwt2d_synthesis_stream': (I, [P, L, I, P, P, I, L, I, I, I, I, P, P, P, P, I, I, I, P]),
diff --git a/pytorch_wavelets_amd/csrc/wl_api_common.h b/pytorch_wavelets_amd/csrc/wl_api_common.h
--- a/pytorch_wavelets_amd/csrc/wl_api_common.h
+++ b/pytorch_wavelets_amd/csrc/wl_api_common.h
@@ -51,6 +51,7 @@
     int64_t planes; int nlev;
     WlBanks taps; int L, mode;
     int strips, hints; float* scratch; int* tstate; void* stream;
+    const float* lat_hint; int* verdict;
 };
 
 #define WL_DISPATCH_DTYPE(dtype, ...)                      \
diff --git a/pytorch_wavelets_amd/csrc/wl_idwt_rows.h b/pytorch_wavelets_amd/csrc/wl_idwt_rows.h
--- a/pytorch_wavelets_amd/csrc/wl_idwt_rows.h
+++ b/pytorch_wavelets_amd/csrc/wl_idwt_rows.h
@@ -15,6 +15,7 @@
 #define WL_ITICK() 0ull
 #endif
 #define WL_IROWS_CHUNK 1024
+#define WL_IROWS_HINT_FLOATS 5
 
 struct WlIRowsLevel {
     int Kh, Kw;
@@ -59,6 +60,8 @@
     int per;
     int guard;
     const float* lat;
+    float hint[WL_IROWS_HINT_FLOATS];
+    int* verdict;
 };
 
 struct WlIRowsSched {
@@ -82,13 +85,14 @@
 };
 
 #ifndef WL_IROWS_LAT_MIN
-#define WL_IROWS_LAT_MIN 8
+#define WL_IROWS_LAT_MIN 10
 #endif
 template <typename T, int LT, int LAT = 0, int PER = 0>
 struct WlSfbRows {
     typedef WlIRowsArgs<T> Args;
     static const int kThreads = 64 * WL_IROWS_WAVES;
     static const int kMinWaves = 7;
+    static_assert(LAT == 0 || LAT == 1 || (LAT == 2 && LT == 8), "the self-guarded form exists for 8 taps");
     static const int HL = LT / 2;
     static const int WARM = HL - 1;
     static const int SZ = (int)sizeof(T);
@@ -254,9 +258,10 @@
     struct __attribute__((packed, aligned(sizeof(T)), may_alias)) WlPairT { T a, b; };
     static const int NP = (HL + 1) / 2;
     static const int NW = HL > 1 ? HL - 1 : 1;
+    template <int BODY>
     struct Wave {
-        wl_v2 gw0[HL], gw1[LAT ? 1 : HL], gh0[LAT ? 1 : HL], gh1[LAT ? 1 : HL];
-        wl_v2 lt[LAT ? HL : 1];
+        wl_v2 gw0[HL], gw1[BODY ? 1 : HL], gh0[BODY ? 1 : HL], gh1[BODY ? 1 : HL];
+        wl_v2 lt[BODY ? HL : 1];
         int coff;
         int coff_ll;
         int ycol1;
@@ -276,7 +281,8 @@
             v[i] = wl_v2{(float)*reinterpret_cast<const T*>(p + 2 * i * SZ), (float)*reinterpret_cast<const T*>(p + (2 * i + 1) * SZ)};
         if (HL & 1) v[NP - 1] = wl_v2{(float)*reinterpret_cast<const T*>(p + (HL - 1) * SZ), 0.f};
     }
-    static WL_DEV void row_syn(const WlIRowsLevel& g, const Wave& R, const char* smem, int k, wl_v2& na, wl_v2& nb) {
+    template <int BODY>
+    static WL_DEV void row_syn(const WlIRowsLevel& g, const Wave<BODY>& R, const char* smem, int k, wl_v2& na, wl_v2& nb) {
         int rll = g.src_off[0] + (k & R.llmask) * g.ll_pitch;
         if (PER && g.head_off >= 0 && k >= g.Kh) rll = g.head_off + (k - g.Kh) * g.ll_pitch;
         const int rb = (k & (g.dma_rows - 1)) * g.rbytes;
@@ -287,7 +293,7 @@
         load_coeffs(smem + (g.src_off[3] + rb + R.coff), vhh);
         na = wl_pk_mul_x(R.gw0[HL - 1], vll[0]);
         nb = wl_pk_mul_x(R.gw0[HL - 1], vlh[0]);
-        if constexpr (LAT != 0) {
+        if constexpr (BODY != 0) {
             wl_qmf_syn_fma<0>(na, R.gw0[0], vhl[0]);
             wl_qmf_syn_fma<0>(nb, R.gw0[0], vhh[0]);
 #pragma unroll
@@ -303,11 +309,11 @@
             }
             return;
         }
-        wl_pk_fma_x(na, R.gw1[LAT ? 0 : HL - 1], vhl[0]);
-        wl_pk_fma_x(nb, R.gw1[LAT ? 0 : HL - 1], vhh[0]);
+        wl_pk_fma_x(na, R.gw1[BODY ? 0 : HL - 1], vhl[0]);
+        wl_pk_fma_x(nb, R.gw1[BODY ? 0 : HL - 1], vhh[0]);
 #pragma unroll
         for (int u = 1; u < HL; ++u) {
-            const int t = LAT ? 0 : HL - 1 - u;
+            const int t = BODY ? 0 : HL - 1 - u;
             if (u & 1) {
                 wl_pk_fma_y(na, R.gw0[t], vll[u / 2]); wl_pk_fma_y(nb, R.gw0[t], vlh[u / 2]);
                 wl_pk_fma_y(na, R.gw1[t], vhl[u / 2]); wl_pk_fma_y(nb, R.gw1[t], vhh[u / 2]);
@@ -317,7 +323,7 @@
             }
         }
     }
-    static WL_DEV void lat_feed(const Wave& R, wl_v2 (&S)[NW], wl_v2 a, wl_v2 b, wl_v2& y0, wl_v2& y1) {
+    static WL_DEV void lat_feed(const Wave<1>& R, wl_v2 (&S)[NW], wl_v2 a, wl_v2 b, wl_v2& y0, wl_v2& y1) {
         wl_v2 q = wl_fma_s<0, 1>(a, R.lt[HL - 1], b);
         wl_v2 p = wl_fma_s<0, 0>(b, R.lt[HL - 1], a);
 #pragma unroll
@@ -331,20 +337,20 @@
         y0 = wl_v2{p.x, q.x}; y1 = wl_v2{p.y, q.y};
     }
     template <int OFF, int NE>
-    static WL_DEV void col_syn(const Wave& R, const wl_v2 (&ea)[NE], const wl_v2 (&eb)[NE], wl_v2& y0, wl_v2& y1) {
+    static WL_DEV void col_syn(const Wave<0>& R, const wl_v2 (&ea)[NE], const wl_v2 (&eb)[NE], wl_v2& y0, wl_v2& y1) {
         y0 = wl_pk_mul_x(R.gh0[0], ea[OFF + HL - 1]); y1 = wl_pk_mul_y(R.gh0[0], ea[OFF + HL - 1]);
         wl_pk_fma_x(y0, R.gh1[0], eb[OFF + HL - 1]);
         wl_pk_fma_y(y1, R.gh1[0], eb[OFF + HL - 1]);
 #pragma unroll
         for (int t = 1; t < HL; ++t) {
-            wl_pk_fma_x(y0, R.gh0[LAT ? 0 : t], ea[OFF + HL - 1 - t]);
-            wl_pk_fma_y(y1, R.gh0[LAT ? 0 : t], ea[OFF + HL - 1 - t]);
-            wl_pk_fma_x(y0, R.gh1[LAT ? 0 : t], eb[OFF + HL - 1 - t]);
-            wl_pk_fma_y(y1, R.gh1[LAT ? 0 : t], eb[OFF + HL - 1 - t]);
-        }
-    }
-    template <int j>
-    static WL_DEV void emit_per(const Wave& R, char* smem, int m, wl_v2 y0, wl_v2 y1) {
+            wl_pk_fma_x(y0, R.gh0[t], ea[OFF + HL - 1 - t]);
+            wl_pk_fma_y(y1, R.gh0[t], ea[OFF + HL - 1 - t]);
+            wl_pk_fma_x(y0, R.gh1[t], eb[OFF + HL - 1 - t]);
+            wl_pk_fma_y(y1, R.gh1[t], eb[OFF + HL - 1 - t]);
+        }
+    }
+    template <int j, int BODY>
+    static WL_DEV void emit_per(const Wave<BODY>& R, char* smem, int m, wl_v2 y0, wl_v2 y1) {
         if (j == 0) {
             if ((WL_IROWS_ABLATE & 1) && y0.x + y0.y + y1.x + y1.y != 1.2345e30f) return;
             int r0 = m + R.rot2;
@@ -382,9 +388,9 @@
             }
         }
     }
-    template <int j>
-    static WL_DEV void emit(const Wave& R, char* smem, int m, wl_v2 y0, wl_v2 y1) {
-        if constexpr (PER != 0) { emit_per<j>(R, smem, m, y0, y1); return; }
+    template <int j, int BODY>
+    static WL_DEV void emit(const Wave<BODY>& R, char* smem, int m, wl_v2 y0, wl_v2 y1) {
+        if constexpr (PER != 0) { emit_per<j, BODY>(R, smem, m, y0, y1); return; }
         if (j == 0) {
             if ((WL_IROWS_ABLATE & 1) && y0.x + y0.y + y1.x + y1.y != 1.2345e30f) return;
             char* r0 = R.yp + ((unsigned)m * R.yrowb + R.ycol);
@@ -417,19 +423,20 @@
         }
     }
 
-    template <int j>
+    template <int j, int BODY>
     static WL_DEV void compute(const Args& a, const WlIRowsSeg& sg, const WlCtx& ctx, int64_t plane, int c0, int lane, int soff) {
         const WlIRowsLevel& g = a.g[j];
         char* const smem = ctx.smem + soff;
         const int c = c0 + lane;
         const bool active = 2 * c < g.OW;
-        Wave R;
-        if constexpr (LAT != 0) {
-            const float gsc = a.lat[1];
+        Wave<BODY> R;
+        if constexpr (BODY != 0) {
+            const float gsc = LAT == 2 ? a.hint[0] : a.lat[1];
 #pragma unroll
             for (int t = 0; t < HL; ++t) {
+                const float tk = LAT == 2 ? a.hint[(1 + t) < WL_IROWS_HINT_FLOATS ? 1 + t : 0] : a.lat[2 + t];
                 R.gw0[t] = wl_uniform_v2(wl_v2{a.g_w_lo[2 * t] * gsc, a.g_w_lo[2 * t + 1] * gsc});
-                R.lt[t] = wl_uniform_v2(wl_v2{a.lat[2 + t], -a.lat[2 + t]});
+                R.lt[t] = wl_uniform_v2(wl_v2{tk, -tk});
             }
         } else {
 #pragma unroll
@@ -492,26 +499,24 @@
             if (!active || (WL_IROWS_ABLATE & 4)) continue;
             const int m = 2 * (k - WARM);
             wl_v2 y0, y1;
-            if constexpr (LAT != 0) {
+            if constexpr (BODY != 0) {
                 wl_v2 na, nb;
                 row_syn(g, R, smem, k, na, nb);
                 lat_feed(R, wa, na, nb, y0, y1);
-                if (k - f0 >= WARM) emit<j>(R, smem, m, y0, y1);
+                if (k - f0 >= WARM) emit<j, BODY>(R, smem, m, y0, y1);
                 if (n == 2) {
                     row_syn(g, R, smem, k + 1, na, nb);
                     lat_feed(R, wa, na, nb, y0, y1);
-                    if (k + 1 - f0 >= WARM) emit<j>(R, smem, m + 2, y0, y1);
-                }
-                continue;
-            }
-            if (n == 2) {
+                    if (k + 1 - f0 >= WARM) emit<j, BODY>(R, smem, m + 2, y0, y1);
+                }
+            } else if (n == 2) {
                 wl_v2 ea[HL + 1], eb[HL + 1];
                 row_syn(g, R, smem, k, ea[HL - 1], eb[HL - 1]);
                 row_syn(g, R, smem, k + 1, ea[HL], eb[HL]);
 #pragma unroll
                 for (int t = 0; t < HL - 1; ++t) { ea[t] = wa[t]; eb[t] = wb[t]; }
-                if (k - f0 >= WARM) { col_syn<0>(R, ea, eb, y0, y1); emit<j>(R, smem, m, y0, y1); }
-                if (k + 1 - f0 >= WARM) { col_syn<1>(R, ea, eb, y0, y1); emit<j>(R, smem, m + 2, y0, y1); }
+                if (k - f0 >= WARM) { col_syn<0>(R, ea, eb, y0, y1); emit<j, BODY>(R, smem, m, y0, y1); }
+                if (k + 1 - f0 >= WARM) { col_syn<1>(R, ea, eb, y0, y1); emit<j, BODY>(R, smem, m + 2, y0, y1); }
 #pragma unroll
                 for (int t = 0; t < HL - 1; ++t) { wa[t] = ea[t + 2]; wb[t] = eb[t + 2]; }
             } else {
@@ -519,7 +524,7 @@
                 row_syn(g, R, smem, k, ea[HL - 1], eb[HL - 1]);
 #pragma unroll
                 for (int t = 0; t < HL - 1; ++t) { ea[t] = wa[t]; eb[t] = wb[t]; }
-                if (k - f0 >= WARM) { col_syn<0>(R, ea, eb, y0, y1); emit<j>(R, smem, m, y0, y1); }
+                if (k - f0 >= WARM) { col_syn<0>(R, ea, eb, y0, y1); emit<j, BODY>(R, smem, m, y0, y1); }
 #pragma unroll
                 for (int t = 0; t < HL - 1; ++t) { wa[t] = ea[t + 1]; wb[t] = eb[t + 1]; }
             }
@@ -550,9 +555,28 @@
             if constexpr (PER != 0) loader_per(a, sg, ctx, plane, lane, arg >> 4, (arg >> 2) & 3, (arg & 3) + 1, soff);
             else loader(a, sg, ctx, plane, lane, arg >> 4, (arg >> 2) & 3, (arg & 3) + 1, soff);
         }
-        else if (lev == 0) compute<0>(a, sg, ctx, plane, arg, lane, soff);
-        else if (lev == 1) compute<1>(a, sg, ctx, plane, arg, lane, soff);
-        else if (lev == 2) compute<2>(a, sg, ctx, plane, arg, lane, soff);
+        else if (lev >= 0) {
+            if constexpr (LAT == 2) {
+                bool holds = wl_taps_qmf(a.g_w_lo, a.g_w_hi, LT) & wl_taps_qmf(a.g_h_lo, a.g_h_hi, LT)
+                           & wl_taps_same(a.g_w_lo, a.g_h_lo, LT) & wl_taps_same(a.g_w_hi, a.g_h_hi, LT);
+                holds = wl_lattice_syn_realises<LT>(a.g_h_lo, a.g_h_hi, a.hint[0], a.hint + 1, SZ == 2 ? 0x1p-12 : 0x1p-22) & holds;
+                const bool lattice = wl_uniform(holds ? 1 : 0) != 0;
+                if (a.verdict && bid == 0 && lev == 0 && arg == 0 && sub == 0 && lane == 0) *a.verdict = lattice ? 1 : 0;
+                if (lattice) {
+                    if (lev == 0) compute<0, 1>(a, sg, ctx, plane, arg, lane, soff);
+                    else if (lev == 1) compute<1, 1>(a, sg, ctx, plane, arg, lane, soff);
+                    else compute<2, 1>(a, sg, ctx, plane, arg, lane, soff);
+                } else {
+                    if (lev == 0) compute<0, 0>(a, sg, ctx, plane, arg, lane, soff);
+                    else if (lev == 1) compute<1, 0>(a, sg, ctx, plane, arg, lane, soff);
+                    else compute<2, 0>(a, sg, ctx, plane, arg, lane, soff);
+                }
+            } else {
+                if (lev == 0) compute<0, LAT>(a, sg, ctx, plane, arg, lane, soff);
+                else if (lev == 1) compute<1, LAT>(a, sg, ctx, plane, arg, lane, soff);
+                else compute<2, LAT>(a, sg, ctx, plane, arg, lane, soff);
+            }
+        }
         else
             for (int hb = 0; hb < sg.nhb; ++hb) if (!(WL_IROWS_ABLATE & 64) || !(hb & 1)) ctx.sync();
     }
diff --git a/pytorch_wavelets_amd/csrc/wl_lattice.h b/pytorch_wavelets_amd/csrc/wl_lattice.h
--- a/pytorch_wavelets_amd/csrc/wl_lattice.h
+++ b/pytorch_wavelets_amd/csrc/wl_lattice.h
@@ -71,6 +71,51 @@
     }
     *g = (float)(-gain);
     return ab(gain) > 1e-30;
+}
+
+template <int L>
+WL_HD bool wl_lattice_syn_realises(const float* lo, const float* hi, float g, const float* T, double tol, double* dev = nullptr) {
+    static_assert(L >= 4 && L % 2 == 0 && L / 2 <= WL_LAT_MAXK, "even tap counts from 4 to 20");
+    const int K = L / 2;
+    double scale = 0.0, worst = 0.0;
+    bool ok = true;
+#pragma unroll
+    for (int t = 0; t < L; ++t) {
+        const double a = lo[t] < 0 ? -(double)lo[t] : (double)lo[t], b = hi[t] < 0 ? -(double)hi[t] : (double)hi[t];
+        ok = ok & (a <= 1e30) & (b <= 1e30);
+        scale = a > scale ? a : scale; scale = b > scale ? b : scale;
+    }
+    ok = ok & (scale > 0.0);
+    const double bound = tol * scale, gd = (double)g;
+    double Td[K];
+#pragma unroll
+    for (int k = 0; k < K; ++k) Td[k] = (double)T[k];
+#pragma unroll
+    for (int in = 0; in < 2; ++in) {
+        double S[K > 1 ? K - 1 : 1];
+#pragma unroll
+        for (int k = 0; k < K - 1; ++k) S[k] = 0.0;
+#pragma unroll
+        for (int t = 0; t < K; ++t) {
+            const double a = t == 0 && in == 0 ? 1.0 : 0.0, b = t == 0 && in == 1 ? 1.0 : 0.0;
+            double q = Td[K - 1] * a - b, p = a + Td[K - 1] * b;
+#pragma unroll
+            for (int k = K - 1; k >= 1; --k) {
+                const double d = S[k - 1];
+                S[k - 1] = q;
+                const double n = p - Td[k - 1] * d;
+                q = d + Td[k - 1] * p;
+                p = n;
+            }
+            const double w0 = in ? (double)hi[2 * t] : (double)lo[2 * t], w1 = in ? (double)hi[2 * t + 1] : (double)lo[2 * t + 1];
+            double e0 = gd * p - w0, e1 = gd * q - w1;
+            e0 = e0 < 0 ? -e0 : e0; e1 = e1 < 0 ? -e1 : e1;
+            ok = ok & (e0 <= bound) & (e1 <= bound);
+            worst = !(e0 <= worst) ? e0 : worst; worst = !(e1 <= worst) ? e1 : worst;
+        }
+    }
+    if (dev) *dev = scale > 0.0 ? worst / scale : worst;
+    return ok;
 }
 
 template <int HI, int NZ> WL_DEV wl_v2 wl_fma_s(wl_v2 w, wl_v2 pair, wl_v2 z) {
diff --git a/pytorch_wavelets_amd/csrc/wl_rows_api.inc b/pytorch_wavelets_amd/csrc/wl_rows_api.inc
--- a/pytorch_wavelets_amd/csrc/wl_rows_api.inc
+++ b/pytorch_wavelets_amd/csrc/wl_rows_api.inc
@@ -556,12 +556,17 @@
     a.g_h_lo = (const float*)r.taps.h_lo; a.g_h_hi = (const float*)r.taps.h_hi;
     a.NC = planes;
     a.guard = guard; a.lat = lat;
+    for (int i = 0; i < WL_IROWS_HINT_FLOATS; ++i) a.hint[i] = LAT == 2 && r.lat_hint && i <= LT / 2 ? r.lat_hint[i] : 0.f;
+    a.verdict = LAT == 2 ? r.verdict : nullptr;
     if (what == 1) return 0;
     return what == 2 ? wl_launch_armed<K>(a, units + ncut, (size_t)off, r.stream) : wl_launch<K>(a, units + ncut, (size_t)off, r.stream);
 }
 
 template <typename T, int LT, int PER = 0>
 static int wl_sfb_rows_pick(const WlSfbPyrReq& r) {
+    if constexpr (LT == 8) {
+        if (r.lat_hint) return wl_sfb_rows_launch<T, LT, 2, PER>(r);
+    }
     if constexpr (LT >= WL_IROWS_LAT_MIN) {
         if ((r.hints & 3) == 3 && r.scratch)
             return wl_lattice_launch<LT>([&](int guard, int what) { return wl_sfb_rows_launch<T, LT, 0, PER>(r, r.scratch, guard, what); },
@@ -582,11 +587,12 @@
 #undef WL_CASE
 }
 
-extern "C" int wl_dwt2d_synthesis_fused_ex(const void* yl, int64_t yl_plane_stride, int yl_row_stride, int yl_h, int yl_w,
-                                           const void* const* yh, const int* Kh, const int* Kw, void* y, int dtype,
-                                           int64_t planes, int nlev, const void* g_w_lo, const void* g_w_hi,
-                                           const void* g_h_lo, const void* g_h_hi, int L, int mode, int strips,
-                                           void* tap_scratch, int* tap_state, void* stream) {
+extern "C" int wl_dwt2d_synthesis_fused_hint(const void* yl, int64_t yl_plane_stride, int yl_row_stride, int yl_h, int yl_w,
+                                             const void* const* yh, const int* Kh, const int* Kw, void* y, int dtype,
+                                             int64_t planes, int nlev, const void* g_w_lo, const void* g_w_hi,
+                                             const void* g_h_lo, const void* g_h_hi, int L, int mode, int strips,
+                                             void* tap_scratch, int* tap_state, const float* lattice_hint, void* lattice_verdict,
+                                             void* stream) {
     if (wl_mode_to_ext(mode) < 0) return WL_ERR_MODE;
     if (planes < 0 || yl_h < 1 || yl_w < 1) return WL_ERR_SHAPE;
     if (L < 1 || L > WL_MAX_TAPS) return WL_ERR_TAPS;
@@ -598,8 +604,32 @@
     if (strips == 0 && 8 * planes < 3 * wl_num_cus()) return WL_ERR_UNSUPPORTED;
     if (planes == 0) return 0;
     const WlSfbPyrReq r = {yl, yl_plane_stride, yl_row_stride, yl_h, yl_w, yh, Kh, Kw, y, planes, nlev,
-                           {g_w_lo, g_w_hi, g_h_lo, g_h_hi}, L, mode, strips, hints, (float*)tap_scratch, tap_state, stream};
+                           {g_w_lo, g_w_hi, g_h_lo, g_h_hi}, L, mode, strips, hints, (float*)tap_scratch, tap_state, stream,
+                           L == 8 ? lattice_hint : nullptr, (int*)lattice_verdict};
     WL_DISPATCH_FLOAT(dtype, return wl_sfb_rows_dispatch<T>(r));
+}
+
+extern "C" int wl_dwt2d_synthesis_fused_ex(const void* yl, int64_t yl_plane_stride, int yl_row_stride, int yl_h, int yl_w,
+                                           const void* const* yh, const int* Kh, const int* Kw, void* y, int dtype,
+                                           int64_t planes, int nlev, const void* g_w_lo, const void* g_w_hi,
+                                           const void* g_h_lo, const void* g_h_hi, int L, int mode, int strips,
+                                           void* tap_scratch, int* tap_state, void* stream) {
+    return wl_dwt2d_synthesis_fused_hint(yl, yl_plane_stride, yl_row_stride, yl_h, yl_w, yh, Kh, Kw, y, dtype, planes, nlev,
+                                         g_w_lo, g_w_hi, g_h_lo, g_h_hi, L, mode, strips, tap_scratch, tap_state, nullptr, nullptr, stream);
+}
+
+extern "C" int wl_lattice_factor_host(const float* lo, const float* hi, int L, int syn, double tol, float* out) {
+    if (!lo || !hi || !out || L < 4 || L > 2 * WL_LAT_MAXK || L % 2) return WL_ERR_TAPS;
+    float g = 0.f, T[WL_LAT_MAXK];
+    bool ok = false;
+    switch (L) {
+#define WL_CASE(LT_) case LT_: ok = wl_lattice_factor<LT_>(lo, hi, tol, &g, T, syn != 0); break
+        WL_CASE(4); WL_CASE(6); WL_CASE(8); WL_CASE(10); WL_CASE(12); WL_CASE(14); WL_CASE(16); WL_CASE(18); WL_CASE(20);
+#undef WL_CASE
+    }
+    out[0] = ok ? g : 0.f;
+    for (int k = 0; k < L / 2; ++k) out[1 + k] = ok ? T[k] : 0.f;
+    return ok ? 1 : 0;
 }
 
 extern "C" int wl_dwt2d_synthesis_fused(const void* yl, int64_t yl_plane_stride, int yl_row_stride, int yl_h, int yl_w,
diff --git a/pytorch_wavelets_amd/ops.py b/pytorch_wavelets_amd/ops.py
--- a/pytorch_wavelets_amd/ops.py
+++ b/pytorch_wavelets_amd/ops.py
@@ -229,7 +229,7 @@
     ent = cache.get(key) if cache is not None else None
     if ent is None:
         taps = tuple(_taps(b, ref) for b in bufs)
-        scratch = _new_tap_scratch(ref.device) if L >= min(ROWS_LATTICE_MIN, IROWS_LATTICE_MIN) and (STRIP_LATTICE or ROWS_LATTICE) else None
+        scratch = _new_tap_scratch(ref.device) if L >= min(ROWS_LATTICE_MIN, SCRATCH_MIN_TAPS) and (STRIP_LATTICE or ROWS_LATTICE) else None
         ent = [taps, scratch, ctypes.c_int(0)]
         if cache is not None:
             cache[key] = ent
@@ -238,6 +238,35 @@
 
 def _new_tap_scratch(device):
     return torch.empty(TAP_SCRATCH_FLOATS, dtype=torch.float32, device=device)
+
+
+_LATTICE_HINTS = {}
+_LATTICE_HINTS_MAX = 256
+ONE_LAUNCH_VERDICT = None
+
+
+def _lattice_hint(lo, hi, ref):
+    two = ref.element_size() == 2
+    try:
+        key = tuple((b.data_ptr(), b._version, b.dtype, b.device, tuple(b.shape)) for b in (lo, hi)) + (two,)
+    except (RuntimeError, AttributeError):
+        key = tuple((b.data_ptr(), -1, b.dtype, b.device, tuple(b.shape)) for b in (lo, hi)) + (two,)
+    ent = _LATTICE_HINTS.get(key)
+    if ent is None:
+        L = lo.numel()
+        fl, fh = (_taps(b, ref).cpu().contiguous() for b in (lo, hi))
+        out = (ctypes.c_float * (L // 2 + 1))()
+        pf = ctypes.POINTER(ctypes.c_float)
+        rc = _backend().wl_lattice_factor_host(ctypes.cast(fl.data_ptr(), pf), ctypes.cast(fh.data_ptr(), pf), L, 1,
+                                               2.0 ** -12 if two else 2.0 ** -22, out)
+        if rc != 1:
+            if rc < 0:
+                _lib.check(rc, 'wl_lattice_factor_host')
+            out = (ctypes.c_float * (L // 2 + 1))(*([float('nan')] * (L // 2 + 1)))
+        if len(_LATTICE_HINTS) >= _LATTICE_HINTS_MAX:
+            _LATTICE_HINTS.clear()
+        ent = _LATTICE_HINTS[key] = out
+    return ent
 
 
 def _launch_taps(bufs, ref, L, syn, hinted):
@@ -460,6 +489,14 @@
     ptrs = (ctypes.c_void_p * nlev)(*[t.data_ptr() for t in yh])
     khs = (ctypes.c_int * nlev)(*[t.shape[3] for t in yh])
     kws = (ctypes.c_int * nlev)(*[t.shape[4] for t in yh])
+    if lattice and L == IROWS_ONE_LAUNCH_TAPS:
+        hint = _lattice_hint(g_h_lo, g_h_hi, yl)
+        verdict = ONE_LAUNCH_VERDICT.data_ptr() if ONE_LAUNCH_VERDICT is not None and ONE_LAUNCH_VERDICT.device == yl.device else None
+        if _declined(key, 'wl_dwt2d_synthesis_fused_hint', yl, yl.data_ptr(), yl_ps, yl_rs, kh, kw, ptrs, khs, kws,
+                     y.data_ptr(), _DTYPES[yl.dtype], N * C, nlev, gwl.data_ptr(), gwh.data_ptr(), ghl.data_ptr(),
+                     ghh.data_ptr(), L, mode, strips | _fused_hint_bits(same, qmf), None, None, hint, verdict, _stream(yl)):
+            return None
+        return y
     if _declined(key, 'wl_dwt2d_synthesis_fused_ex', yl, yl.data_ptr(), yl_ps, yl_rs, kh, kw, ptrs, khs, kws,
                  y.data_ptr(), _DTYPES[yl.dtype], N * C, nlev, gwl.data_ptr(), gwh.data_ptr(), ghl.data_ptr(),
                  ghh.data_ptr(), L, mode, strips | _fused_hint_bits(same, qmf), scratch, ctypes.byref(tstate), _stream(yl)):
@@ -475,6 +512,8 @@
 LATTICE_MIN_ELEMS = 40000000
 LATTICE_MIN_ELEMS_ML = 16000000
 IROWS_LATTICE_MIN = 8
+IROWS_ONE_LAUNCH_TAPS = 8
+SCRATCH_MIN_TAPS = 10
 
 
 IROWS_F16_MAXL = 8
```

After: 300,500 Mpixels/s. No clear change (-0.1%).
